# stoneMo/DeepAVFusion

Hardware: AMD Instinct MI355X
Metric: AV-pairs/sec, DeepAVFusion ViT-B pre-training step (224px + 10s audio, image mask 0.75) (higher is better)
Workload: dtype bf16; 1 GPU; AVMAE(DeepAVFusion base) fwd+bwd+allreduce+AdamW, B=64/GPU, 224x224 RGB + (128,640) log-mel, masks 0.75/0.8, fusion attn_ratio 0.25 mlp_ratio 1.0; global_batch=64, parallelism=dp1, graph=True

## Files before the change

deepavfusion_amd/_lib.py:

```python
from __future__ import annotations

import ctypes as C
import os

import torch

_HERE = os.path.dirname(os.path.abspath(__file__))
LIB_PATH = os.path.join(_HERE, 'libdavfusion_hip.so')

_p, _i, _l, _f, _sz = C.c_void_p, C.c_int, C.c_long, C.c_float, C.c_size_t

ABI_VERSION = 9

SIGNATURES = {
    'dav_abi_version': [],
    'dav_build_flags': [],
    'dav_last_error_string': [],
    'dav_tune': [_i, _i],
    'dav_gemm_nt_bf16': [_p, _p, _i, _i, _i, _i, _i, _p, _p, _i, _p, _i, _p, _i, _p, _p, _p, _i, _i, _p, _p, _i, _i, _i, _f, _i, _p],
    'dav_gemm_nt_ln_bf16': [_p, _p, _i, _i, _i, _i, _i, _p, _p, _i, _p, _i, _p, _i, _p, _p, _p, _i, _i, _p, _p, _i, _i, _i, _f, _i, _p, _p],
    'dav_ln_fold_grouped': [_p, _i, _p],
    'dav_rowstats_cast': [_p, _l, _i, _i, _i, _p, _p, _p],
    'dav_layernorm_bwd_twin': [_p, _l, _p, _i, _p, _l, _p, _i, _i, _i, _f, _p, _p, _p, _p,
                               _p, _l, _i, _p, _l, _p, _l,
                               _p, _l, _i, _p, _l, _p, _l,
                               _p, _p, _p, _p, _sz, _p],
    'dav_nt_issue_log': [_i, _p, _i],
    'dav_nt_tune_set': [_p, _i],
    'dav_gemm_tn_bf16': [_p, _p, _i, _i, _i, _i, _i, _p, _p, _p, _i, _i, _p, _i, _p],
    'dav_gemm_tn_grouped_bf16': [_p, _i, _p],
    'dav_gemm_tn_gang_workspace_bytes': [_p, _i],
    'dav_gemm_tn_gang_bf16': [_p, _i, _p, _sz, _p],
    'dav_gemm_tn_grouped_bf16_gated': [_p, _i, _p, _p],
    'dav_gemm_tn_gang_bf16_gated': [_p, _i, _p, _sz, _p, _p],
    'dav_attn_fwd': [_p, _p, _p, _p, _p, _i, _i, _i, _i, _i, _i, _l, _i, _l, _i, _l, _i, _l, _i, _f, _p],
    'dav_attn_bwd': [_p] * 10 + [_i] * 6 + [_l, _i] * 8 + [_f, _p],
    'dav_attn_bwd_part': [_p] * 10 + [_i] * 6 + [_l, _i] * 8 + [_f, _i, _p],
    'dav_add_cast': [_p, _p, _p, _p, _l, _p],
    'dav_attn_bwd_ctx': [_p] * 10 + [_i] * 6 + [_l, _i] * 8 + [_f, _i, _i, _p],
    'dav_attn_bias_fwd': [_p, _p, _p, _p, _p, _i, _i, _i, _i, _i, _i, _l, _i, _l, _i, _l, _i, _l, _i, _f, _p, _i, _i, _p],
    'dav_attn_bias_bwd': [_p] * 10 + [_i] * 6 + [_l, _i] * 8 + [_f, _p, _i, _i, _p, _i, _p],
    'dav_attn_drop_fwd': [_p, _p, _p, _p, _p, _i, _i, _i, _i, _i, _i, _l, _i, _l, _i, _l, _i, _l, _i, _f, _p, _i, _f, _p],
    'dav_attn_drop_bwd': [_p] * 10 + [_i] * 6 + [_l, _i] * 8 + [_f, _p, _i, _f, _i, _i, _p],
    'dav_window_unfold': [_p, _i, _p, _i, _i, _i, _i, _i, _i, _f, _p, _i, _p],
    'dav_window_fold': [_p, _p, _p, _i, _i, _i, _i, _i, _i, _f, _p, _p],
    'dav_relpos_bias_build': [_p, _p, _p, _i, _i, _i, _i, _i, _f, _p, _p],
    'dav_relpos_bias_bwd': [_p, _p, _i, _i, _i, _i, _i, _i, _p, _p],
    'dav_layernorm_fwd': [_p, _l, _i, _p, _l, _i, _i, _i, _p, _p, _f, _p, _p, _p, _p, _p],
    'dav_layernorm_bwd': [_p, _l, _i, _p, _l, _i, _i, _i, _p, _p, _p, _p, _p,
                          _p, _l, _i, _p, _l, _p, _l,
                          _p, _l, _i, _p, _l, _p, _l,
                          _p, _p, _p, _sz, _p],
    'dav_layernorm_bwd_workspace_bytes': [_i, _i],
    'dav_layernorm_bwd_reduce_grouped': [_p, _i, _p],
    'dav_mask_build': [_p, _i, _i, _i, _p, _p, _p, _p, _p, _p],
    'dav_patch_gather': [_p, _i, _i, _i, _i, _p, _i, _p, _p],
    'dav_patch_gather3d': [_p, _i, _i, _i, _i, _i, _i, _p, _i, _p, _p],
    'dav_unshuffle_fwd': [_p, _p, _p, _p, _i, _i, _i, _i, _p, _l, _i, _p],
    'dav_rows_gather_cast': [_p, _l, _i, _p, _i, _i, _i, _p, _p],
    'dav_rows_axpy': [_p, _p, _p, _i, _i, _i, _p, _p],
    'dav_rows_scale_cast': [_p, _p, _i, _i, _i, _p, _p],
    'dav_dropout_rows': [_p, _i, _p, _p, _f, _p, _i, _i, _i, _p, _i, _p],
    'dav_unshuffle_bwd_reduce': [_p, _l, _i, _p, _i, _i, _i, _i, _p, _p, _p],
    'dav_patch_mse_fwd': [_p, _p, _p, _i, _i, _i, _i, _i, _p, _p, _p, _p, _p, _p],
    'dav_patch_mse_bwd': [_p, _p, _p, _p, _p, _p, _p, _i, _i, _i, _i, _p, _p],
    'dav_pair_expand': [_p, _p, _i, _i, _i, _i, _p, _p],
    'dav_pair_reduce': [_p, _i, _i, _i, _i, _p, _p, _p],
    'dav_cast_bf16': [_p, _p, _l, _p],
    'dav_cast_transpose_bf16': [_p, _p, _i, _i, _p],
    'dav_l2norm_workspace_bytes': [_l],
    'dav_l2norm': [_p, _l, _f, _p, _p, _sz, _p],
    'dav_gemm_nt_f32': [_p, _p, _i, _i, _i, _i, _i, _p, _p, _i, _p, _i, _p, _i, _p, _p, _p, _i, _p, _p, _i, _i, _i, _f, _i, _p],
    'dav_gemm_tn_f32': [_p, _p, _i, _i, _i, _i, _i, _p, _p, _p, _i, _i, _p, _p],
    'dav_attn_fwd_f32': [_p, _p, _p, _p, _p, _i, _i, _i, _i, _i, _i, _l, _i, _l, _i, _l, _i, _l, _i, _f, _p],
    'dav_attn_bwd_f32': [_p] * 10 + [_i] * 6 + [_l, _i] * 8 + [_f, _i, _p],
    'dav_attn_bias_fwd_f32': [_p, _p, _p, _p, _p, _i, _i, _i, _i, _i, _i, _l, _i, _l, _i, _l, _i, _l, _i, _f, _p, _i, _i, _p],
    'dav_attn_bias_bwd_f32': [_p] * 10 + [_i] * 6 + [_l, _i] * 8 + [_f, _p, _i, _i, _p, _i, _p],
    'dav_attn_drop_fwd_f32': [_p, _p, _p, _p, _p, _i, _i, _i, _i, _i, _i, _l, _i, _l, _i, _l, _i, _l, _i, _f, _p, _i, _f, _p],
    'dav_attn_drop_bwd_f32': [_p] * 10 + [_i] * 6 + [_l, _i] * 8 + [_f, _p, _i, _f, _i, _p],
    'dav_patch_gather_f32': [_p, _i, _i, _i, _i, _i, _i, _p, _i, _p, _p],
    'dav_rows_gather_f32': [_p, _l, _i, _p, _i, _i, _i, _p, _l, _p],
    'dav_pair_expand_f32': [_p, _p, _i, _i, _i, _i, _p, _p],
    'dav_pair_reduce_f32': [_p, _i, _i, _i, _i, _p, _p, _p],
    'dav_patch_mse_bwd_f32': [_p, _p, _p, _p, _p, _p, _p, _i, _i, _i, _i, _p, _p],
    'dav_add_f32': [_p, _p, _p, _l, _p],
    'dav_logmel': [_p, _i, _i, _i, _i, _i, _p, _p, _p, _p, _p, _p, _f, _i, _i, _p, _p],
    'dav_log10_eps': [_p, _f, _l, _p, _p],
    'dav_mean_l2n_f32': [_p, _i, _i, _i, _l, _l, _p, _p],
    'dav_knn_topk_f32': [_p] * 6 + [_i, _i, _i, _i, _l, _l, _i, _i, _i, _p, _p, _p, _sz, _p],
    'dav_knn_topk_wide_f32': [_p] * 6 + [_i, _i, _i, _i, _l, _l, _i, _i, _i, _p, _p, _p, _sz, _p],
    'dav_knn_vote_f32': [_p, _p, _i, _i, _i, _i, _p, _p, _i, _i, _p, _i, _p, _p, _p],
    'dav_frame_transform_u8': [_p, _i, _i, _i, _p, _i, _f, _f, _f, _f, _f, _f, _p, _p],
    'dav_wave_resample_tile': [_i, _i, _i],
    'dav_wave_resample': [_p, _i, _i, _i, _l, _p, _i, _i, _i, _p, _i, _p, _i, _l, _p],
    'dav_batch_begin': [_i],
    'dav_batch_lane': [],
    'dav_batch_region': [_i],
    'dav_batch_skip': [_i],
    'dav_batch_suspend': [_i],
    'dav_batch_end': [],
    'dav_batch_abort': [],
    'dav_batch_stats': [_p, _p],
    'dav_adamw_flat': [_p, _p, _p, _p, _p, _l, _p, _p, _i, _f, _f, _f, _p, _f, _p, _i, _p, _p, _p],
    'dav_step_guard': [_p, _p, _p, _f, _f, _p, _p, _p],
    'dav_cast_transpose_grouped': [_p, _i, _p],
}

class DavLnReduce(C.Structure):
    _fields_ = [('workspace', C.c_void_p), ('dgamma', C.c_void_p), ('dbeta', C.c_void_p), ('rows', C.c_int), ('D', C.c_int)]


class DavNtLn(C.Structure):
    _fields_ = [('stats', C.c_void_p), ('stats2', C.c_void_p), ('A2', C.c_void_p), ('ln_c', C.c_void_p), ('eps', C.c_float),
                ('a_r0', C.c_int), ('a_r1', C.c_int), ('stats_out', C.c_void_p), ('twin_out', C.c_void_p), ('ld_twin', C.c_int)]


class DavLnFold(C.Structure):
    _fields_ = [('w', C.c_void_p), ('gamma', C.c_void_p), ('beta', C.c_void_p), ('bias', C.c_void_p),
                ('w_ln_bf16', C.c_void_p), ('ln_c', C.c_void_p), ('ln_d', C.c_void_p), ('N', C.c_int), ('K', C.c_int)]


class DavTranspose(C.Structure):
    _fields_ = [('x', C.c_void_p), ('y_bf16', C.c_void_p), ('R', C.c_int), ('C', C.c_int)]


class DavTnProblem(C.Structure):
    _fields_ = [('A', C.c_void_p), ('B', C.c_void_p), ('C', C.c_void_p), ('bias_grad', C.c_void_p),
                ('Mc', C.c_int), ('N', C.c_int), ('K', C.c_int), ('lda', C.c_int), ('ldb', C.c_int), ('ldc', C.c_int),
                ('a_rowmap', C.c_int * 3), ('b_rowmap', C.c_int * 3), ('flags', C.c_int)]


ERRORS = {-1: 'bad shape', -2: 'unsupported dtype', -3: 'insufficient workspace', -4: 'HIP error', -5: 'misaligned pointer/stride'}

_lib = None


def load():
    global _lib
    if _lib is not None:
        return _lib
    if not os.path.exists(LIB_PATH):
        raise RuntimeError(f'{LIB_PATH} is missing: the DeepAVFusion HIP kernels are not built '
                           '(run __graft_entry__.build() or make -C deepavfusion_amd/csrc). There is no CPU fallback.')
    lib = C.CDLL(LIB_PATH)
    for name, argtypes in SIGNATURES.items():
        fn = getattr(lib, name)
        fn.argtypes = argtypes
        fn.restype = _sz if name.endswith('workspace_bytes') else (C.c_char_p if name == 'dav_last_error_string' else _i)
    if lib.dav_abi_version() != ABI_VERSION:
        raise RuntimeError('libdavfusion_hip.so ABI version mismatch')
    _lib = lib
    load_nt_tuning(NT_TUNING_PATH)
    return lib


def kernel_source_hash():
    import glob
    import hashlib
    here = os.path.dirname(os.path.abspath(__file__))
    h = hashlib.sha1()
    for f in sorted(glob.glob(os.path.join(here, 'csrc', '*.hip')) + glob.glob(os.path.join(here, 'csrc', '*.h'))) + [os.path.join(here, 'tuning', 'nt_gfx950.json')]:
        h.update(os.path.basename(f).encode())
        h.update(open(f, 'rb').read())
    return h.hexdigest()[:16]


NT_TUNING_PATH = os.environ.get('DAV_NT_TUNE_FILE') or os.path.join(os.path.dirname(os.path.abspath(__file__)), 'tuning', 'nt_gfx950.json')


def load_nt_tuning(path):
    if os.environ.get('DAV_NT_TUNE', '1') == '0' or not path or not os.path.exists(path):
        _lib.dav_nt_tune_set(None, 0)
        return 0
    import json
    blob = []
    for e in json.load(open(path))['entries']:
        blob += [int(e['cfg']), int(e['b_kn']), len(e['problems'])]
        for q in e['problems']:
            blob += [int(x) for x in q]
    arr = (C.c_int * len(blob))(*blob)
    n = _lib.dav_nt_tune_set(arr, len(blob))
    if n < 0:
        raise RuntimeError(f'{path}: malformed tuning table ({ERRORS.get(n, n)})')
    return n


def check(code: int, what: str):
    if code != 0:
        detail = ''
        if code == -4 and _lib is not None:
            detail = f" ({_lib.dav_last_error_string().decode()})"
        raise RuntimeError(f'{what} failed: {ERRORS.get(code, code)}{detail}')
```

deepavfusion_amd/autograd_bridge.py:

```python
from __future__ import annotations

import os

import torch

from . import engine as E
from . import ops
from .ops import F32


_SIDE_STREAMS = {}


def _streams(dev):
    main = torch.cuda.current_stream(dev)
    if os.environ.get('DAV_STREAMS', '1') == '0':
        return main, main, main
    key = dev.index if dev.index is not None else torch.cuda.current_device()
    if key not in _SIDE_STREAMS:
        _SIDE_STREAMS[key] = (torch.cuda.Stream(dev), torch.cuda.Stream(dev))
    sa, sf = _SIDE_STREAMS[key]
    return main, sa, sf


# ... 270 lines not shown
            E.flush_wgrads()
        if layer_cb is not None and l > 0:
            layer_cb(l)
    E.patch_embed_bwd(vis, t['t_pi'], g_i, g_ib)
    E.patch_embed_bwd(enc.audio, t['t_pa'], g_a, g_ab)
    E.gbuf(enc.fusion_tokens).add_(g_f.sum(dim=0, keepdim=True))
    E._ready(enc.fusion_tokens)


class _EncoderFn(torch.autograd.Function):
    @staticmethod
    def forward(ctx, enc, image, audio, ik32, ak32, return_embs, need_tape, *params):
        ctx.set_materialize_grads(False)
        with E.ln_fuse_for(need_tape):
            _, f32s, embs, tape = encoder_fwd(enc, image, audio, ik32, ak32, want_f32=True, collect_embs=return_embs)
        ctx.enc, ctx.tape = enc, (tape if need_tape else None)
        B = image.shape[0]
        outs = [x.view(B, -1, x.shape[-1]) for x in f32s]
        flat_embs = [e for tri in embs for e in tri]
        ctx.mark_non_differentiable(*flat_embs)
        return (*outs, *flat_embs)

    @staticmethod
    def backward(ctx, gi, ga, gf, *_):
        if ctx.tape is None:
            raise RuntimeError('backward through DeepAVFusion.forward called without a saved tape')
        c = lambda g: None if g is None else g.contiguous().view(-1, g.shape[-1])
        encoder_bwd(ctx.enc, ctx.tape, dxi32=c(gi), dxa32=c(ga), dxf32=c(gf))
        ctx.tape = None
        return (None,) * (7 + len(ctx.enc._param_list))


def encoder_apply(enc, image, audio, image_ids_keep, audio_ids_keep, return_embs):
    enc._param_list = [p for p in enc.parameters()]
    need_tape = torch.is_grad_enabled() and any(p.requires_grad for p in enc._param_list)
    out = _EncoderFn.apply(enc, _f32c(image), _f32c(audio), _ids32(image_ids_keep), _ids32(audio_ids_keep),
                           bool(return_embs), need_tape, *enc._param_list)
    if not return_embs:
        return out[0], out[1], out[2]
    rest = out[3:]
    embs = [tuple(rest[3 * i:3 * i + 3]) for i in range(len(rest) // 3)]
    return out[0], out[1], out[2], embs


class _PatchTokensFn(torch.autograd.Function):
    @staticmethod
    def forward(ctx, vit, x, ids32, *params):
        ctx.set_materialize_grads(False)
        tok, tape = E.patch_embed_fwd(vit, x, ids32)
        ctx.vit, ctx.tape = vit, tape
        return tok

    @staticmethod
    def backward(ctx, g):
        E.patch_embed_bwd(ctx.vit, ctx.tape, g.contiguous(), None)
        return (None,) * (3 + 2)


def patch_tokens(vit, x, ids_keep):
    return _PatchTokensFn.apply(vit, _f32c(x), _ids32(ids_keep), vit.patch_embed.proj.weight, vit.patch_embed.proj.bias)


class _CrossAttentionFn(torch.autograd.Function):

    @staticmethod
    def forward(ctx, ca, x1, x2, *params):
        ctx.set_materialize_grads(False)
        B, N1, D = x1.shape
        N2 = x2.shape[1]
        x1b, x2b = E.to_bf16(x1.reshape(B * N1, D)), E.to_bf16(x2.reshape(B * N2, D))
        H, hd = ca.num_heads, D // ca.num_heads
        S = _sampler(ca, 'cross')
        pa, pp = (ca.attn_drop_prob, ca.proj_drop_prob) if ca.training else (0.0, 0.0)
        keep = E.draw_attn_keep(pa, B, H, N1, N2, x1.device, S('attn', (B, H, N1, N2))) if pa > 0.0 else None
        ctx.pm = E.draw_keep(pp, B * N1, D, x1.device, S('proj', (B, N1, D), lambda m: m.reshape(B * N1, D))) if pp > 0.0 else None
        c = E._cross_fwd_seq(ca, x1b, None, N1, x2b, N2, B, D, ca.num_heads, x1.device, keep=keep)
        out = E.lin_fwd(ca.proj, c['o'], B * N1)
        if ctx.pm is not None:
            E._drop(out, ctx.pm, B, N1, D)
        ctx.ca, ctx.c, ctx.x1b, ctx.x2b, ctx.dims, ctx.np = ca, c, x1b, x2b, (B, N1, N2, D), len(params)
        q = c['q'].view(B, N1, H, hd).permute(0, 2, 1, 3).float()
        k = c['kv'].view(B, N2, 2, H, hd)[:, :, 0].permute(0, 2, 1, 3).float()
        attn = torch.exp((q @ k.transpose(-2, -1)) * ca.scale - c['lse'].unsqueeze(-1))
        if keep is not None:
            attn = attn * keep[0][..., :N2].float() * keep[2]
        ctx.mark_non_differentiable(attn)
        return out.view(B, N1, D), attn

    @staticmethod
    def backward(ctx, g, _g_attn):
        B, N1, N2, D = ctx.dims
        ca = ctx.ca
        with E.deferred_wgrads():
            gb = E.to_bf16(g.contiguous().view(B * N1, D))
            if ctx.pm is not None:
                gb = gb.clone() if gb.data_ptr() == g.data_ptr() else gb
                E._drop(gb, ctx.pm, B, N1, D)
            do = E.lin_bwd(ca.proj, gb, ctx.c['o'], B * N1)
            dx1 = torch.empty(B * N1, D, dtype=E.BF16, device=g.device)
            dx2 = E._cross_bwd_seq(ca, ctx.c, do, ctx.x1b, None, N1, ctx.x2b, N2, B, D, ca.num_heads, dx1, None)
        return (None, dx1.float().view(B, N1, D), dx2.float().view(B, N2, D)) + (None,) * ctx.np


def cross_attention(ca, x1, x2):
    params = [p for p in ca.parameters()]
    c = lambda x: x.to(dtype=F32).contiguous()
    return _CrossAttentionFn.apply(ca, c(x1), c(x2), *params)


class _SwinBlockFn(torch.autograd.Function):
    @staticmethod
    def forward(ctx, blk, xcat, nF, *params):
        ctx.set_materialize_grads(False)
        out, tape = E.swin_block_fwd(blk, xcat, nF)
        ctx.blk, ctx.tape, ctx.np = blk, tape, len(params)
        return out

    @staticmethod
    def backward(ctx, g):
        with E.deferred_wgrads():
            dx, _ = E.swin_block_bwd(ctx.blk, ctx.tape, g.contiguous(), None)
        return (None, dx, None) + (None,) * ctx.np


def swin_block_apply(blk, x, x_fusion):
    nF = x_fusion.shape[1]
    xcat = torch.cat([x_fusion.to(dtype=F32), x.to(dtype=F32)], dim=1).contiguous()
    out = _SwinBlockFn.apply(blk, xcat, nF, *list(blk.parameters()))
    return out[:, nF:], out[:, :nF]


class _FusionBlockFn(torch.autograd.Function):
    @staticmethod
    def forward(ctx, fb, xmm, xv, xa, *params):
        ctx.set_materialize_grads(False)
        out, tape = E.fusion_block_fwd(fb, xmm, xv, xa, fb.num_heads, getattr(fb, 'fusion_tkns', None),
                                       drop_path_scales(fb, fb, xmm.shape[0], xmm.device, 'fusion'),
                                       fusion_drops(fb, fb, xmm.shape[0], xmm.shape[1], xv.shape[1], xa.shape[1], xmm.device, 'fusion'))
        ctx.fb, ctx.tape, ctx.np = fb, tape, len(params)
        return out

    @staticmethod
    def backward(ctx, g):
        with E.deferred_wgrads():
            dx_f, dx_i, dx_a = E.fusion_block_bwd(ctx.fb, ctx.tape, g.contiguous(), None)
        return (None, dx_f, dx_i, dx_a) + (None,) * ctx.np


def fusion_block(fb, xmm, xv, xa):
    c = lambda x: x.to(dtype=F32).contiguous()
    return _FusionBlockFn.apply(fb, c(xmm), c(xv), c(xa), *list(fb.parameters()))


def avmae_fwd(model, image, audio, noise_i, noise_a):
    with E.fold_scope(model):
        return _avmae_fwd(model, image, audio, noise_i, noise_a)


def _avmae_fwd(model, image, audio, noise_i, noise_a):
    enc = model.encoder
    B = image.shape[0]
    Li, La = model.image_gs[0] * model.image_gs[1], model.audio_gs[0] * model.audio_gs[1]
    nki, nka = int(Li * (1 - model.image_mask_ratio)), int(La * (1 - model.audio_mask_ratio))
    ik, im, ir, ik32, ir32 = ops.mask_build(noise_i, nki)
    ak, am, ar, ak32, ar32 = ops.mask_build(noise_a, nka)
    (xi_b, xa_b, xf_b), _, _, t_enc = encoder_fwd(enc, image, audio, ik32, ak32)
    nF = enc.fusion_tokens.shape[1]
    dec_i, dec_a = model.decoder('image'), model.decoder('audio')
    main, sa, _ = _streams(image.device)
    lanes = t_enc['lanes']
    if lanes:
        with E.batch() as bt:
            bt.lane()
            pred_i, t_di = E.decoder_fwd(dec_i, xi_b, xf_b, ir32, B, nki, nF)
            loss_i, t_li = E.loss_fwd(image, pred_i, im, model.image_norm_loss)
            bt.lane()
            pred_a, t_da = E.decoder_fwd(dec_a, xa_b, xf_b, ar32, B, nka, nF)
            loss_a, t_la = E.loss_fwd(audio, pred_a, am, model.audio_norm_loss)
    else:
        si = main
        sa.wait_stream(main)
        if si is not main:
            si.wait_stream(main)

        def chain(dec, x_b, r32, nk, target, mask, norm_loss):
            pred, t_d = yield from E.decoder_fwd_steps(dec, x_b, xf_b, r32, B, nk, nF)
            loss, t_l = E.loss_fwd(target, pred, mask, norm_loss)
            return pred, t_d, loss, t_l
        (pred_a, t_da, loss_a, t_la), (pred_i, t_di, loss_i, t_li) = paired_steps(
            chain(dec_a, xa_b, ar32, nka, audio, am, model.audio_norm_loss), sa,
            chain(dec_i, xi_b, ir32, nki, image, im, model.image_norm_loss), si, DEC_JOIN)
        main.wait_stream(sa)
        if si is not main:
            main.wait_stream(si)
    tape = dict(image=image, audio=audio, im=im, am=am, ik32=ik32, ak32=ak32, dec_lanes=lanes, t_enc=t_enc, t_di=t_di, t_da=t_da, t_li=t_li,
                t_la=t_la, pred_i=pred_i, pred_a=pred_a, B=B)
    aux = dict(image_ids_keep=ik, image_mask=im, image_ids_restore=ir, audio_ids_keep=ak, audio_mask=am, audio_ids_restore=ar)
    return (loss_i, loss_a, pred_i, pred_a), tape, aux


_DEC_WGRAD_JOINT = True
_ADD_CAST = True


def avmae_bwd(model, t, g_li, g_la, g_pi=None, g_pa=None, layer_cb=None):
    B = t['B']
    dec_i, dec_a = model.decoder('image'), model.decoder('audio')
    main, sa, _ = _streams(t['image'].device)
    if t['dec_lanes']:
        dpi = E.loss_bwd(t['image'], t['pred_i'], t['im'], t['t_li'], g_li)
        dpa = E.loss_bwd(t['audio'], t['pred_a'], t['am'], t['t_la'], g_la)
        if g_pi is not None:
            dpi = (dpi.float() + g_pi.reshape(dpi.shape)).to(E.BF16)
        if g_pa is not None:
            dpa = (dpa.float() + g_pa.reshape(dpa.shape)).to(E.BF16)
        with E.deferred_wgrads():
            with E.batch() as bt:
                bt.lane()
                dxi_b, dxf_i = E.decoder_bwd(dec_i, t['t_di'], dpi, t['ik32'], B)
                bt.lane()
                dxa_b, dxf_a = E.decoder_bwd(dec_a, t['t_da'], dpa, t['ak32'], B)
    elif _DEC_WGRAD_JOINT and sa is not main:
        with E.deferred_wgrads():
            si = main
            sa.wait_stream(main)
            if si is not main:
                si.wait_stream(main)

            def chain(dec, target, pred, mask, t_l, g_l, g_p, t_d, k32):
                dp = E.loss_bwd(target, pred, mask, t_l, g_l)
                if g_p is not None:
                    dp = (dp.float() + g_p.reshape(dp.shape)).to(E.BF16)
                return (yield from E.decoder_bwd_steps(dec, t_d, dp, k32, B))
            (dxa_b, dxf_a), (dxi_b, dxf_i) = paired_steps(
                chain(dec_a, t['audio'], t['pred_a'], t['am'], t['t_la'], g_la, g_pa, t['t_da'], t['ak32']), sa,
                chain(dec_i, t['image'], t['pred_i'], t['im'], t['t_li'], g_li, g_pi, t['t_di'], t['ik32']), si, DEC_JOIN)
            main.wait_stream(sa)
            if si is not main:
                main.wait_stream(si)
            E.deferred_operands_to(main)
    else:
        sa.wait_stream(main)
        with torch.cuda.stream(sa), E.deferred_wgrads():
            dpa = E.loss_bwd(t['audio'], t['pred_a'], t['am'], t['t_la'], g_la)
            if g_pa is not None:
                dpa = (dpa.float() + g_pa.reshape(dpa.shape)).to(E.BF16)
            dxa_b, dxf_a = E.decoder_bwd(dec_a, t['t_da'], dpa, t['ak32'], B)
        with E.deferred_wgrads():
            dpi = E.loss_bwd(t['image'], t['pred_i'], t['im'], t['t_li'], g_li)
            if g_pi is not None:
                dpi = (dpi.float() + g_pi.reshape(dpi.shape)).to(E.BF16)
            dxi_b, dxf_i = E.decoder_bwd(dec_i, t['t_di'], dpi, t['ik32'], B)
        main.wait_stream(sa)
    dxf32 = dxf_i.float() + dxf_a.float()
    if layer_cb is not None:
        layer_cb(len(model.encoder.fusion_blocks))
    encoder_bwd(model.encoder, t['t_enc'], dxi_b=dxi_b, dxa_b=dxa_b, dxf32=dxf32, layer_cb=layer_cb)


class _AVMAEFn(torch.autograd.Function):
    @staticmethod
    def forward(ctx, model, image, audio, noise_i, noise_a, need_tape, *params):
        ctx.set_materialize_grads(False)
        with E.ln_fuse_for(need_tape):
            outs, tape, aux = avmae_fwd(model, image, audio, noise_i, noise_a)
        ctx.model, ctx.tape, ctx.np = model, (tape if need_tape else None), len(params)
        model._last_masks = aux
        return outs

    @staticmethod
    def backward(ctx, g_li, g_la, g_pi, g_pa):
        z = lambda g: g.contiguous() if g is not None else torch.zeros((), dtype=F32, device=ctx.tape['image'].device)
        avmae_bwd(ctx.model, ctx.tape, z(g_li), z(g_la), g_pi, g_pa)
        ctx.tape = None
        return (None,) * (6 + ctx.np)


def avmae_apply(model, image, audio, noise_image=None, noise_audio=None):
    B, dev = image.shape[0], image.device
    Li, La = model.image_gs[0] * model.image_gs[1], model.audio_gs[0] * model.audio_gs[1]
    if noise_image is None:
        noise_image = torch.rand(B, Li, device=dev)
    if noise_audio is None:
        noise_audio = torch.rand(B, La, device=dev)
    params = getattr(model, '_param_list', None)
    if params is None:
        params = model._param_list = [p for p in model.parameters()]
    need_tape = torch.is_grad_enabled() and any(p.requires_grad for p in params)
    return _AVMAEFn.apply(model, _f32c(image), _f32c(audio), _f32c(noise_image), _f32c(noise_audio), need_tape, *params)
```

deepavfusion_amd/engine.py:

```python
from __future__ import annotations

import os
from typing import Callable, Dict, List, NamedTuple, Optional

import torch

from . import ops
from .ops import F32

BF16 = torch.bfloat16
PRECISION = 'bf16'


def set_precision(p: str):
    global BF16, PRECISION
    if p not in ('bf16', 'fp32'):
        raise ValueError(p)
    PRECISION = p
    BF16 = torch.float32 if p == 'fp32' else torch.bfloat16

_GRAD_READY: Optional[Callable[[torch.nn.Parameter], None]] = None


def set_grad_ready_hook(fn: Optional[Callable[[torch.nn.Parameter], None]]):
# ... 343 lines not shown
            return self.own.__exit__(et, ev, tb)
        if _BATCH is not None and et is None:
            ops.batch_region(False)
        return False


WGRAD_GANG = os.environ.get('DAV_WGRAD_GANG', '1') != '0'
WGRAD_GANG_MIN_TILES = 512
WGRAD_MERGE = int(os.environ.get('DAV_WGRAD_MERGE', '0'))
WGRAD_FLUSH_LAYERS = None


WGRAD_EAGER_DP_MERGE = 3


def wgrad_flush_due(layer: int, depth: int) -> bool:
    if not WGRAD_GANG or layer == 0 or layer in (WGRAD_FLUSH_LAYERS or ()):
        return True
    if WGRAD_MERGE > 0:
        return (depth - layer) % WGRAD_MERGE == 0
    return _GRAD_READY is not None and WGRAD_FLUSH_LAYERS is None and (depth - layer) % WGRAD_EAGER_DP_MERGE == 0


_DEFERRED = None
_DEFERRED_LN = None
_DEFERRED_LN_READY = []


class deferred_wgrads:
    def __enter__(self):
        global _DEFERRED, _DEFERRED_LN
        self.prev = (_DEFERRED, _DEFERRED_LN)
        _DEFERRED, _DEFERRED_LN = [], []
        return self

    def __exit__(self, *exc):
        global _DEFERRED, _DEFERRED_LN
        if exc[0] is None:
            flush_wgrads()
        _DEFERRED, _DEFERRED_LN = self.prev


_OVERWRITE = None


def wgrad_overwrite_begin(gate=None):
    global _OVERWRITE
    _OVERWRITE = dict(written=set(), touched=set(), params={}, gate=gate)


def wgrad_overwrite_end():
    global _OVERWRITE
    st, _OVERWRITE = _OVERWRITE, None
    return list(st['params'].values()) if st else []


def deferred_operands_to(stream):
    for pr in (_DEFERRED or []):
        for k in ('A', 'B'):
            t = pr.get(k)
            if torch.is_tensor(t) and t.is_cuda:
                t.record_stream(stream)
    for item in (_DEFERRED_LN or []):
        if torch.is_tensor(item[0]) and item[0].is_cuda:
            item[0].record_stream(stream)


def flush_wgrads():
    if _DEFERRED_LN:
        items = list(_DEFERRED_LN)
        del _DEFERRED_LN[:]
        ops.layernorm_bwd_reduce_grouped(items)
        for pair in _DEFERRED_LN_READY:
            _ready(*pair)
        del _DEFERRED_LN_READY[:]
    if not _DEFERRED:
        return
    probs = list(_DEFERRED)
    del _DEFERRED[:]
    while probs:
        seen, now, later = set(), [], []
        for pr in probs:
            key = pr['C'].data_ptr()
            (later if key in seen else now).append(pr)
            seen.add(key)
        now.sort(key=lambda pr: -pr['Mc'])
        gate = _OVERWRITE['gate'] if _OVERWRITE is not None else None
        gated = {} if gate is None else {'gate': gate}
        gang = WGRAD_GANG and PRECISION == 'bf16' and (sum(-(-pr['N'] // 256) * -(-pr['K'] // 256) for pr in now) >= WGRAD_GANG_MIN_TILES
                                                       or any(pr['Mc'] % 64 for pr in now))
        if _OVERWRITE is not None:
            for pr in now:
                key = pr['C'].data_ptr()
                pr['overwrite'] = bool(pr.get('weight') is not None and key not in _OVERWRITE['written'] and key not in _OVERWRITE['touched'])
                if gate is not None and (pr['A'].dtype == F32 or (not gang and pr['Mc'] % 64)):
                    pr['overwrite'] = False
                _OVERWRITE['written'].add(key)
                if pr.get('weight') is None:
                    _OVERWRITE['touched'].add(pr.get('gbase', key))
                if pr['overwrite']:
                    _OVERWRITE['params'][id(pr['weight'])] = pr['weight']
        if gang:
            ops.gemm_tn_gang(now, **gated)
        else:
            grouped = [pr for pr in now if pr['Mc'] % 64 == 0 or pr['A'].dtype == F32]
            if grouped:
                ops.gemm_tn_grouped(grouped, **gated)
            for pr in now:
                if pr['Mc'] % 64 and pr['A'].dtype != F32:
                    ops.gemm_tn(pr['A'], pr['B'], pr['Mc'], pr['N'], pr['K'], pr['C'], lda=pr['lda'], ldb=pr['ldb'], ldc=pr['ldc'],
                                a_rowmap=pr.get('a_rowmap'), b_rowmap=pr.get('b_rowmap'), beta=0 if pr.get('overwrite') else 1,
                                bias_grad=pr.get('bias_grad'))
        for pr in now:
            _ready(*pr['ready'])
        probs = later


def ln_fwd(norm, x0, x1, B, eps=None, want_f32=False, want_bf16=True):
    D = norm.weight.shape[0]
    r0 = x0.shape[1] if x0 is not None else 0
    r1 = x1.shape[1] if x1 is not None else 0
    if x0 is None:
        x0, r0, x1, r1 = x1, r1, None, 0
    dev = x0.device
    M = B * (r0 + r1)
    y = _e((M, D), BF16, dev) if want_bf16 else None
    y32 = _e((M, D), F32, dev) if want_f32 else None
    if PRECISION == 'fp32' and y is not None and y32 is not None:
        y32 = y
    mean, rstd = _e((M,), F32, dev), _e((M,), F32, dev)
    ops.layernorm_fwd(x0, r0 * D, r0, x1, r1 * D, r1, B, D, norm.weight, norm.bias, norm.eps if eps is None else eps,
                      y, y32, mean, rstd)
    return y, y32, (mean, rstd)


def ln_bwd(norm, x0, x1, B, stats, dy_bf16=None, dy_f32=None, *, dx0=None, acc0=0, res0=None, dx0_bf16=None,
           dx1=None, acc1=0, res1=None, dx1_bf16=None):
    D = norm.weight.shape[0]
    r0 = x0.shape[1] if x0 is not None else 0
    r1 = x1.shape[1] if x1 is not None else 0
    if x0 is None:
        x0, r0, x1, r1 = x1, r1, None, 0
        dx0, acc0, res0, dx0_bf16, dx1, acc1, res1, dx1_bf16 = dx1, acc1, res1, dx1_bf16, None, 0, None, None
    ops.layernorm_bwd(x0, r0 * D, r0, x1, r1 * D, r1, B, D, dy_bf16, dy_f32, norm.weight, stats[0], stats[1],
                      dx0, r0 * D, acc0, res0, r0 * D, dx0_bf16, r0 * D,
                      dx1, r1 * D, acc1, res1, r1 * D, dx1_bf16, r1 * D,
                      gbuf(norm.weight), gbuf(norm.bias), defer=_DEFERRED_LN)
    if _DEFERRED_LN is None:
        _ready(norm.weight, norm.bias)
    else:
        _DEFERRED_LN_READY.append((norm.weight, norm.bias))


def lin_fwd(lin, a, M, *, a_rowmap=None, lda=None, act=0, res=None, res_rowmap=None, out=None, out_bf16=False,
            c_rowmap=None, ldc=None, C2=None, c2_mode=0, w_col_off=0, k=None, use_bias=True):
    W = wcache(lin.weight)
    N, Kfull = W.shape
    K = Kfull if k is None else k
    dev = a.device
    if out is None:
        out = _e((M, N), BF16 if out_bf16 else F32, dev)
    Bw = W if w_col_off == 0 else W.view(-1)[w_col_off:]
    ops.gemm_nt(a, Bw, M, N, K, lda=lda if lda is not None else K, ldb=Kfull, a_rowmap=a_rowmap,
                bias=lin.bias if use_bias else None, act=act, res=res, ldres=N, res_rowmap=res_rowmap,
                C_out=out, ldc=ldc if ldc is not None else N, c_bf16=out.dtype == BF16, c_rowmap=c_rowmap,
                C2=C2, ldc2=N, c2_mode=c2_mode)
    return out


def lin_bwd(lin, dy, a, M, *, dy_rowmap=None, a_rowmap=None, lda=None, need_dx=True, gelu_aux=None, dx=None, dx_bf16=True,
            dx_rowmap=None, dx_beta=0, dx_C2=None, dx_c2_mode=0, w_col_off=0, k=None, use_bias=True, final=True,
            dx_res=None, dx_res_rowmap=None, wgrad=True):
    W = wcache(lin.weight)
    N, Kfull = W.shape
    K = Kfull if k is None else k
    dev = dy.device
    if need_dx:
        if dx is None:
            dx = _e((M, K), BF16 if dx_bf16 else F32, dev)
        if N % 64 == 0 or PRECISION == 'fp32':
            Bt, ldb, variant = (W if w_col_off == 0 else W.view(-1)[w_col_off:]), Kfull, 1 << 12
        else:
            WT = wcache_t(lin.weight)
            Bt, ldb, variant = (WT if w_col_off == 0 else WT[w_col_off:]), N, 0
        ops.gemm_nt(dy, Bt, M, K, N, lda=N, ldb=ldb, a_rowmap=dy_rowmap, act=3 if gelu_aux is not None else 0,
                    aux=gelu_aux, ldaux=K, res=dx_res, ldres=K, res_rowmap=dx_res_rowmap,
                    C_out=dx, ldc=K, c_bf16=dx.dtype == BF16, c_rowmap=dx_rowmap, beta=dx_beta,
                    C2=dx_C2, ldc2=K, c2_mode=dx_c2_mode, variant=variant)
    if wgrad:
        lin_wgrad(lin, dy, a, M, dy_rowmap=dy_rowmap, a_rowmap=a_rowmap, lda=lda, w_col_off=w_col_off, k=k, use_bias=use_bias, final=final)
    return dx


def lin_wgrad(lin, dy, a, M, *, dy_rowmap=None, a_rowmap=None, lda=None, w_col_off=0, k=None, use_bias=True, final=True):
    N, Kfull = lin.weight.shape[0], lin.weight.numel() // lin.weight.shape[0]
    K = Kfull if k is None else k
    gw = gbuf(lin.weight)
    gwv = gw.view(N, -1)
    Cw = gwv if w_col_off == 0 else gwv.view(-1)[w_col_off:]
    gb = gbuf(lin.bias) if (use_bias and lin.bias is not None) else None
    if _DEFERRED is not None and N % 8 == 0 and K % 8 == 0 and (M % 64 == 0 or (WGRAD_GANG and PRECISION == 'bf16')):
        _DEFERRED.append(dict(A=dy, B=a, Mc=M, N=N, K=K, C=Cw, lda=N, ldb=lda if lda is not None else K, ldc=Kfull,
                              a_rowmap=dy_rowmap, b_rowmap=a_rowmap, bias_grad=gb,
                              ready=(lin.weight, lin.bias) if final else (),
                              gbase=gwv.data_ptr(),
                              weight=lin.weight if (w_col_off == 0 and K == Kfull) else None))
        return
    if _OVERWRITE is not None:
        _OVERWRITE['touched'].add(gwv.data_ptr())
    ops.gemm_tn(dy, a, M, N, K, Cw, lda=N, ldb=lda if lda is not None else K, ldc=Kfull, a_rowmap=dy_rowmap,
                b_rowmap=a_rowmap, beta=1, bias_grad=gb)
    if final:
        _ready(lin.weight, lin.bias)


def lin_fwd_ln(lin, norm, eps, t0, M, *, t1=None, r0=0, r1=0, a_rowmap=None, act=0, out_bf16=True, out=None, C2=None, c2_mode=0):
    f = ln_fold(lin, norm)
    N, K = f.wl.shape
    if out is None:
        out = _e((M, N), BF16 if out_bf16 else F32, f.wl.device)
    ln = dict(stats=t0[1], ln_c=f.c, eps=eps)
    if t1 is not None:
        ln.update(A2=t1[0], stats2=t1[1], a_r0=r0, a_r1=r1)
    ops.gemm_nt_ln(t0[0], f.wl, M, N, K, ln=ln, a_rowmap=a_rowmap, bias=f.d, act=act, C_out=out, c_bf16=out.dtype == BF16,
                   C2=C2, ldc2=N, c2_mode=c2_mode)
    return out


def lin_fwd_tw(lin, a, M, res, *, res_rowmap=None, res_rows=None, out=None, tw=None, c_rowmap=None, C2=None, c2_mode=0, rows_out=None):
    W = wcache(lin.weight)
    N, K = W.shape
    dev = a.device
    R = M if rows_out is None else rows_out
    if out is None:
        out = _e((R, N), F32, dev)
    if tw is None:
        tw = (_e((R, N), BF16, dev), _e((R, N // 64, 2), F32, dev))
    ops.gemm_nt_ln(a, W, M, N, K, prod=dict(stats_out=tw[1], twin_out=tw[0], ld_twin=N), bias=lin.bias, res=res, ldres=N,
                   res_rowmap=res_rowmap, res_rows=res_rows, C_out=out, c_rowmap=c_rowmap, C2=C2, ldc2=N, c2_mode=c2_mode)
    return out, tw


def ln_bwd_tw(norm, eps, t0, r0, t1, r1, B, dy_bf16=None, dy_f32=None, *, h_out=None, dx0=None, acc0=0, res0=None, dx0_bf16=None,
              dx1=None, acc1=0, res1=None, dx1_bf16=None):
    D = norm.weight.shape[0]
    if t0 is None:
        t0, r0, t1, r1 = t1, r1, None, 0
        dx0, acc0, res0, dx0_bf16, dx1, acc1, res1, dx1_bf16 = dx1, acc1, res1, dx1_bf16, None, 0, None, None
    ops.layernorm_bwd_twin(t0[0], r0 * D, t0[1], r0, t1[0] if t1 is not None else None, r1 * D, t1[1] if t1 is not None else None, r1,
                           B, D, eps, dy_bf16, dy_f32, norm.weight, norm.bias,
                           dx0, r0 * D, acc0, res0, r0 * D, dx0_bf16, r0 * D,
                           dx1, r1 * D, acc1, res1, r1 * D, dx1_bf16, r1 * D,
                           h_out=h_out, dgamma=gbuf(norm.weight), dbeta=gbuf(norm.bias), defer=_DEFERRED_LN)
    if _DEFERRED_LN is None:
        _ready(norm.weight, norm.bias)
    else:
        _DEFERRED_LN_READY.append((norm.weight, norm.bias))


class AttnView(NamedTuple):
    t: torch.Tensor
    off: int
    bs: int
    rs: int


def cols(buf, rows, c0=0, r0=0):
    ld = buf.shape[1]
    return AttnView(buf, r0 * ld + c0, rows * ld, ld)


def qkv_cols(qkv, rows, D, r0=0):
    return cols(qkv, rows, 0, r0), cols(qkv, rows, D), cols(qkv, rows, 2 * D)


def _attn_ptr(name, v, B, N, width, r0_is=0):
    t, off, bs, rs = v
    ok = t.dim() == 2 and t.is_contiguous() and off >= 0 and rs == t.shape[1] and rs > 0 and bs % rs == 0 and t.shape[0] == B * (bs // rs)
    if ok:
        r0, c0 = divmod(off, rs)
        ok = c0 + width <= rs and r0 + N <= bs // rs and (not r0_is or r0 == r0_is)
    if not ok:
        raise ValueError(f'attention operand {name}: (off, bs, rs) = {tuple(v[1:])} into {tuple(t.shape)} (contiguous: {t.is_contiguous()}) '
                         f'does not hold {B} x {N} rows of {width} columns' + (f' from row {r0_is}' if r0_is else ''))
    return t.data_ptr() + t.element_size() * off


def attention_fwd(q, k, v, B, H, Nq, Nk, dqk, dv, scale, keep=None, bias=None):
    ptrs = (_attn_ptr('q', q, B, Nq, H * dqk), _attn_ptr('k', k, B, Nk, H * dqk), _attn_ptr('v', v, B, Nk, H * dv))
    dev = q.t.device
    O = _e((B * Nq, H * dv), BF16, dev)
    LSE = _e((B, H, Nq), F32, dev)
    ops.hold(q.t, k.t, v.t)
    args = (*ptrs, O, LSE, B, H, Nq, Nk, dqk, dv, q.bs, q.rs, k.bs, k.rs, v.bs, v.rs, Nq * H * dv, H * dv, scale)
    if keep is not None:
        ops.attn_drop_fwd(*args, *keep)
    elif bias is not None:
        ops.attn_bias_fwd(*args, *bias)
    else:
        ops.attn_fwd(*args)
    return O, LSE


_ATTN_CTX = True


def attention_bwd(q, k, v, O, dO, LSE, dq, dk, dv_, B, H, Nq, Nk, dqk, dv, scale, part=3, Delta=None, dq_ctx_rows=0, keep=None,
                  bias=None, dS=None):
    ptrs = (_attn_ptr('q', q, B, Nq, H * dqk), _attn_ptr('k', k, B, Nk, H * dqk), _attn_ptr('v', v, B, Nk, H * dv),
            _attn_ptr('dq', dq, B, Nq, H * dqk, dq_ctx_rows), _attn_ptr('dk', dk, B, Nk, H * dqk), _attn_ptr('dv', dv_, B, Nk, H * dv))
    if Delta is None:
        Delta = torch.empty_like(LSE)
    ops.hold(q.t, k.t, v.t, dq.t, dk.t, dv_.t)
    args = (*ptrs[:3], O, dO, LSE, Delta, *ptrs[3:], B, H, Nq, Nk, dqk, dv, q.bs, q.rs, k.bs, k.rs, v.bs, v.rs,
            Nq * H * dv, H * dv, Nq * H * dv, H * dv, dq.bs, dq.rs, dk.bs, dk.rs, dv_.bs, dv_.rs, scale)
    if keep is not None:
        ops.attn_drop_bwd(*args, *keep, part=part, dq_ctx_rows=dq_ctx_rows)
    elif bias is not None:
        ops.attn_bias_bwd(*args, *bias, dS, part=part)
    else:
        ops.attn_bwd(*args, part=part, dq_ctx_rows=dq_ctx_rows)


def to_bf16(x):
    if PRECISION == 'fp32':
        return x.contiguous()
    y = torch.empty(x.shape, dtype=BF16, device=x.device)
    ops.cast_bf16(x.contiguous(), y)
    return y


def draw_attn_keep(p, B, H, Nq, Nk, dev, sample=None):
    ld = (Nk + 31) // 32 * 32
    if sample is None:
        m = (torch.rand((B, H, Nq, ld), device=dev) >= p).to(torch.uint8)
    else:
        m = torch.zeros((B, H, Nq, ld), device=dev, dtype=torch.uint8)
# ... 535 lines not shown
    B, nF, D = x_f.shape
    n2, n3 = x_2.shape[1], x_3.shape[1]
    nS = n3 + n2
    dev, at = x_f.device, fb.attn
    Da = at.q.weight.shape[0]
    hd = Da // heads
    g1, g1b = _mlp_tail_bwd(fb, t, g, gb, B, nF, D, dev)
    dp, dr = t.get('dp'), t.get('dr') or {}
    if dp is not None or 'proj' in dr:
        g1b = _branch_grad(g1, None if dp is None else dp[0], dr.get('proj'), B, nF, D)
    do = lin_bwd(at.proj, g1b, t['o'], B * nF)
    dq, dkv = _e((B * nF, Da), BF16, dev), _e((B * nS, 2 * Da), BF16, dev)
    attention_bwd(cols(t['q'], nF), cols(t['kv'], nS), cols(t['kv'], nS, Da), t['o'], do, t['lse'],
                  cols(dq, nF), cols(dkv, nS), cols(dkv, nS, Da), B, heads, nF, nS, hd, hd, hd ** -0.5, keep=dr.get('attn'))
    dxmm_b = lin_bwd(at.q, dq, t['xmm_b'], B * nF)
    dx3_b = lin_bwd(at.kv, dkv, t['x3_b'], B * n3, dy_rowmap=(n3, nS, 0), final=False)
    dx2_b = lin_bwd(at.kv, dkv, t['x2_b'], B * n2, dy_rowmap=(n2, nS, n3))
    return _input_norms_bwd(fb, t, (fb.norm1_aud, x_2, t['st_2'], dx2_b), (fb.norm1_img, x_3, t['st_3'], dx3_b), dxmm_b, g1, dx_i, dx_a)


def _dense_fwd(fb, x_f, x_i, x_a, heads, dp=None, dr=None):
    dr = dr or {}
    B, nF, D = x_f.shape
    nI, nA = x_i.shape[1], x_a.shape[1]
    dev, at = x_f.device, fb.attn
    Da = at.q.weight.shape[0]
    hd = Da // heads
    xmm_b, xmm32, st_mm = ln_fwd(fb.norm1_mm, None, x_f, B, want_f32=True)
    xi_b, _, st_i = ln_fwd(fb.norm1_img, None, x_i, B)
    xa_b, _, st_a = ln_fwd(fb.norm1_aud, None, x_a, B)
    pa = lin_fwd(at.kv, xa_b, B * nA, k=D)
    pi = lin_fwd(at.kv, xi_b, B * nI, k=D, w_col_off=D, use_bias=False)
    P = nA * nI
    KV = _e((B * P, 2 * Da), BF16, dev)
    ops.pair_expand(pa, pi, B, nA, nI, 2 * Da, KV)
    q = lin_fwd(at.q, xmm_b, B * nF, out_bf16=True)
    scale = (D // heads) ** -0.5
    o, lse = attention_fwd(cols(q, nF), cols(KV, P), cols(KV, P, Da), B, heads, nF, P, hd, hd, scale, keep=dr.get('attn'))
    xmm1 = _res_add(at.proj, o, B * nF, xmm32, B, nF, D, None if dp is None else dp[0], drop=dr.get('proj')).view(B, nF, D)
    out, tt = _mlp_tail_fwd(fb, xmm1, B, nF, D, dev, dp, dr)
    tt.update(arch='dense_mmi', x_f=x_f, x_i=x_i, x_a=x_a, xmm_b=xmm_b, st_mm=st_mm, xi_b=xi_b, st_i=st_i, xa_b=xa_b, st_a=st_a,
              KV=KV, q=q, o=o, lse=lse, heads=heads)
    return out, tt


def _dense_bwd(fb, t, g, gb, *, dx_i=None, dx_a=None):
    x_f, x_i, x_a, heads = t['x_f'], t['x_i'], t['x_a'], t['heads']
    B, nF, D = x_f.shape
    nI, nA = x_i.shape[1], x_a.shape[1]
    P = nA * nI
    dev, at = x_f.device, fb.attn
    Da = at.q.weight.shape[0]
    hd = Da // heads
    g1, g1b = _mlp_tail_bwd(fb, t, g, gb, B, nF, D, dev)
    dp, dr = t.get('dp'), t.get('dr') or {}
    if dp is not None or 'proj' in dr:
        g1b = _branch_grad(g1, None if dp is None else dp[0], dr.get('proj'), B, nF, D)
    do = lin_bwd(at.proj, g1b, t['o'], B * nF)
    dq, dKV = _e((B * nF, Da), BF16, dev), _e((B * P, 2 * Da), BF16, dev)
    scale = (D // heads) ** -0.5
    attention_bwd(cols(t['q'], nF), cols(t['KV'], P), cols(t['KV'], P, Da), t['o'], do, t['lse'],
                  cols(dq, nF), cols(dKV, P), cols(dKV, P, Da), B, heads, nF, P, hd, hd, scale, keep=dr.get('attn'))
    dxmm_b = lin_bwd(at.q, dq, t['xmm_b'], B * nF)
    dpa, dpi = _e((B * nA, 2 * Da), BF16, dev), _e((B * nI, 2 * Da), BF16, dev)
    ops.pair_reduce(dKV, B, nA, nI, 2 * Da, dpa, dpi)
    dxa_b = lin_bwd(at.kv, dpa, t['xa_b'], B * nA, k=D, final=False)
    dxi_b = lin_bwd(at.kv, dpi, t['xi_b'], B * nI, k=D, w_col_off=D, use_bias=False)
    return _input_norms_bwd(fb, t, (fb.norm1_img, x_i, t['st_i'], dxi_b), (fb.norm1_aud, x_a, t['st_a'], dxa_b), dxmm_b, g1, dx_i, dx_a)


FUSION_IDLE_FWD, FUSION_IDLE_BWD = 4, 6



def fusion_block_batchable(fb, dp=None, dr=None):
    return dp is None and not dr and getattr(fb, 'arch', 'factorized_mmi') == 'factorized_mmi'


def fusion_block_fwd(fb, x_f, x_i, x_a, heads, tkns, dp=None, dr=None):
    arch = getattr(fb, 'arch', 'factorized_mmi')
    if arch == 'token':
        return _token_fwd(fb, x_f, x_i, x_a, heads, dp, dr)
    if arch == 'dense_mmi':
        return _dense_fwd(fb, x_f, x_i, x_a, heads, dp, dr)
    return _factorized_fwd(fb, x_f, x_i, x_a, heads, tkns, dp, dr)


def fusion_block_bwd(fb, t, g, gb, *, dx_i=None, dx_a=None):
    arch = t.get('arch', 'factorized_mmi')
    if arch == 'token':
        return _token_bwd(fb, t, g, gb, dx_i=dx_i, dx_a=dx_a)
    if arch == 'dense_mmi':
        return _dense_bwd(fb, t, g, gb, dx_i=dx_i, dx_a=dx_a)
    return _factorized_bwd(fb, t, g, gb, dx_i=dx_i, dx_a=dx_a)


def patch_embed_fwd(vit, img, ids_keep32):
    B, C = img.shape[:2]
    pe = vit.patch_embed
    L = pe.num_patches
    nk = ids_keep32.shape[1] if ids_keep32 is not None else L
    D = vit.embed_dim
    clip = img.dim() == 5
    pt = pe.patch_size[0] if clip else 1
    if not clip:
        H, W = img.shape[2], img.shape[3]
        assert H == pe.img_size[0], f"Input image height ({H}) doesn't match model ({pe.img_size[0]})."
        assert W == pe.img_size[1], f"Input image width ({W}) doesn't match model ({pe.img_size[1]})."
    else:
        got = (img.shape[2] // pt) * (img.shape[3] // 16) * (img.shape[4] // 16)
        if tuple(img.shape[2:]) != tuple(pe.input_size):
            raise RuntimeError(f'The size of tensor a ({got}) must match the size of tensor b ({L}) at non-singleton dimension 1')
    if C != pe.proj.weight.shape[1]:
        raise RuntimeError(f'Given groups=1, weight of size {list(pe.proj.weight.shape)}, expected input{list(img.shape)} to have '
                           f'{pe.proj.weight.shape[1]} channels, but got {C} channels instead')
    if clip and nk != L:
        raise RuntimeError(f'The size of tensor a ({nk}) must match the size of tensor b ({L}) at non-singleton dimension 1')
    K = C * pt * 256
    A = _e((B * nk, K), BF16, img.device)
    ops.patch_gather(img, ids_keep32, nk, A, pt)
    Wb = wcache(pe.proj.weight)
    tok = _e((B, nk, D), F32, img.device)
    pos_by_id = ids_keep32 is not None and not clip
    if ln_fuse_ok(D) and K % 64 == 0:
        tw = (_e((B * nk, D), BF16, img.device), _e((B * nk, D // 64, 2), F32, img.device))
        ops.gemm_nt_ln(A, Wb, B * nk, D, K, prod=dict(stats_out=tw[1], twin_out=tw[0], ld_twin=D), bias=pe.proj.bias, res=vit.pos_embed,
                       ldres=D, res_rows=ids_keep32 if pos_by_id else None, res_rowmap=None if pos_by_id else (L, 0, 0), C_out=tok)
        tw_set(tok, *tw)
    else:
        ops.gemm_nt(A, Wb, B * nk, D, K, bias=pe.proj.bias, res=vit.pos_embed, ldres=D,
                    res_rows=ids_keep32 if pos_by_id else None, res_rowmap=None if pos_by_id else (L, 0, 0), C_out=tok)
    return tok, dict(A=A, nk=nk)


def patch_embed_bwd(vit, t, g, gb):
    pe = vit.patch_embed
    D = vit.embed_dim
    A = t['A']
    M, K = A.shape
    if gb is None:
        gb = to_bf16(g)
    ops.gemm_tn(gb, A, M, D, K, gbuf(pe.proj.weight).view(D, K), beta=1, bias_grad=gbuf(pe.proj.bias))
    _ready(pe.proj.weight, pe.proj.bias)


def drain(steps):
    try:
        while True:
            next(steps)
    except StopIteration as e:
        return e.value


def decoder_fwd(dec, x_b, xf_b, ids_restore32, B, nk, nF):
    return drain(decoder_fwd_steps(dec, x_b, xf_b, ids_restore32, B, nk, nF))


def decoder_fwd_steps(dec, x_b, xf_b, ids_restore32, B, nk, nF):
    L = ids_restore32.shape[1]
    Dd = dec.embed.weight.shape[0]
    dev = x_b.device
    emb = lin_fwd(dec.embed, x_b, B * nk)
    x = _e((B, nF + L, Dd), F32, dev)
    lin_fwd(dec.embed, xf_b, B * nF, out=x, c_rowmap=(nF, nF + L, 0))
    ops.unshuffle_fwd(emb, dec.mask_token, dec.pos_embed, ids_restore32, B, L, nk, Dd, x, (nF + L) * Dd, nF)
    tapes = []
    swin = getattr(dec, 'arch', 'plain') == 'swin'
    for blk in dec.blocks:
        if swin:
            x, bt = swin_block_fwd(blk, x, nF)
        else:
            x, bt = block_fwd(blk, x, None, dec.heads, blk.norm1.eps)
        tapes.append(bt)
        yield
    D_ = Dd
    if not swin and ln_fuse_ok(Dd):
        tw_last = ensure_tw(x)
        pred = lin_fwd_ln(dec.pred, dec.norm, dec.norm.eps, tw_last, B * L, a_rowmap=(L, nF + L, nF), out_bf16=False)
        P = pred.shape[1]
        tape = dict(x_b=x_b, xf_b=xf_b, tapes=tapes, tw_last=tw_last, ln_fused=True, ids_restore32=ids_restore32, nk=nk, nF=nF, L=L)
        return pred.view(B, L, P), tape
    hN = _e((B * L, D_), BF16, dev)
    mean, rstd = _e((B * L,), F32, dev), _e((B * L,), F32, dev)
    xs = x.view(-1)[nF * Dd:]
    ops.layernorm_fwd(xs, (nF + L) * Dd, L, None, 0, 0, B, Dd, dec.norm.weight, dec.norm.bias, dec.norm.eps, hN, None, mean, rstd)
    pred = lin_fwd(dec.pred, hN, B * L)
    P = pred.shape[1]
    tape = dict(x_b=x_b, xf_b=xf_b, x_last=x, tapes=tapes, hN=hN, stN=(mean, rstd), ids_restore32=ids_restore32, nk=nk, nF=nF, L=L)
    return pred.view(B, L, P), tape


def decoder_bwd(dec, t, dpred_b, ids_keep32, B):
    return drain(decoder_bwd_steps(dec, t, dpred_b, ids_keep32, B))


def decoder_bwd_steps(dec, t, dpred_b, ids_keep32, B):
    nk, nF, L = t['nk'], t['nF'], t['L']
    Dd = dec.embed.weight.shape[0]
    dev = dpred_b.device
    fused = t.get('ln_fused', False)
    dhN = lin_bwd(dec.pred, dpred_b, None if fused else t['hN'], B * L, wgrad=not fused)
    g = _e((B, nF + L, Dd), F32, dev)
    gb = _e((B * (nF + L), Dd), BF16, dev)
    g[:, :nF].zero_()
    gb.view(B, nF + L, Dd)[:, :nF].zero_()
    if fused:
        xb, st = t['tw_last']
        hN = _e((B * L, Dd), BF16, dev)
        ops.layernorm_bwd_twin((xb, nF * Dd), (nF + L) * Dd, (st, nF * (Dd // 64) * 2), L, None, 0, None, 0, B, Dd, dec.norm.eps,
                               dhN, None, dec.norm.weight, dec.norm.bias,
                               (g, nF * Dd), (nF + L) * Dd, 0, None, 0, (gb, nF * Dd), (nF + L) * Dd,
                               h_out=hN, dgamma=gbuf(dec.norm.weight), dbeta=gbuf(dec.norm.bias))
        lin_wgrad(dec.pred, dpred_b, hN, B * L)
    else:
        xs = t['x_last'].view(-1)[nF * Dd:]
        ops.layernorm_bwd(xs, (nF + L) * Dd, L, None, 0, 0, B, Dd, dhN, None, dec.norm.weight, t['stN'][0], t['stN'][1],
                          g.view(-1)[nF * Dd:], (nF + L) * Dd, 0, None, 0, gb.view(-1)[nF * Dd:], (nF + L) * Dd,
                          None, 0, 0, None, 0, None, 0, gbuf(dec.norm.weight), gbuf(dec.norm.bias))
    _ready(dec.norm.weight, dec.norm.bias)
    swin = getattr(dec, 'arch', 'plain') == 'swin'
    yield
    for blk, bt in zip(reversed(list(dec.blocks)), reversed(t['tapes'])):
        if swin:
            g, gb = swin_block_bwd(blk, bt, g, gb)
        else:
            g, gb, _ = block_bwd(blk, bt, g, gb)
        yield
    d_emb = _e((B * nk, Dd), BF16, dev)
    d_embf = _e((B * nF, Dd), BF16, dev)
    ops.rows_gather_cast(g, (nF + L) * Dd, nF, ids_keep32, B, nk, Dd, d_emb)
    ops.rows_gather_cast(g, (nF + L) * Dd, 0, None, B, nF, Dd, d_embf)
    ops.unshuffle_bwd_reduce(g, (nF + L) * Dd, nF, t['ids_restore32'], B, L, nk, Dd, gbuf(dec.pos_embed), gbuf(dec.mask_token))
    _ready(dec.pos_embed, dec.mask_token)
    dx_b = lin_bwd(dec.embed, d_emb, t['x_b'], B * nk, final=False)
    dxf_b = lin_bwd(dec.embed, d_embf, t['xf_b'], B * nF)
    return dx_b, dxf_b


LOG2E = 1.4426950408889634


def swin_block_fwd(blk, x, nF):
    B, R, D = x.shape
    L, dev = R - nF, x.device
    heads, nW = blk.num_heads, blk.num_windows
    A = blk.attn.window_area
    N, hd, M, Mw = A + nF, D // heads, B * R, B * nW * (A + nF)
    h1, _, st1 = ln_fwd(blk.norm1, None, x, B)
    seq = _e((Mw, D), BF16, dev)
    ops.window_unfold(h1, blk.rows32, B, nW, A, nF, L, D, 1.0, seq)
    qkv = lin_fwd(blk.attn.qkv, seq, Mw, out_bf16=True)
    nb = nW if blk.attn_mask is not None else 1
    ld = (N + 31) // 32 * 32
    bias = _e((nb, heads, N, ld), F32, dev)
    ops.relpos_bias_build(blk.attn.relative_position_bias_table, blk.index32, blk.attn_mask, nb, heads, A, N, ld,
                          1.0 if PRECISION == 'fp32' else LOG2E, bias)
    o, lse = attention_fwd(*qkv_cols(qkv, N, D), B * nW, heads, N, N, hd, hd, blk.attn.scale, bias=(bias, nb, ld))
    t = lin_fwd(blk.attn.proj, o, Mw)
    x1 = _e((B, R, D), F32, dev)
    ops.window_fold(t, blk.inv32, x, B, nW, A, nF, L, D, 1.0 / nW, x1)
    h2, _, st2 = ln_fwd(blk.norm2, None, x1, B)
    Hd = blk.mlp.fc1.weight.shape[0]
    z = _e((M, Hd), BF16, dev)
    u = lin_fwd(blk.mlp.fc1, h2, M, act=1, out_bf16=True, C2=z, c2_mode=4)
    x2 = _res_add(blk.mlp.fc2, u, M, x1, B, R, D, None).view(B, R, D)
    tape = dict(x=x, nF=nF, h1=h1, st1=st1, seq=seq, qkv=qkv, bias=bias, nb=nb, ld=ld, o=o, lse=lse, x1=x1, h2=h2, st2=st2, z=z, u=u)
    return x2, tape


def swin_block_bwd(blk, t, g2, g2b=None):
    x, nF = t['x'], t['nF']
    B, R, D = x.shape
    L, dev = R - nF, x.device
    heads, nW = blk.num_heads, blk.num_windows
    A = blk.attn.window_area
    N, hd, M, Mw = A + nF, D // heads, B * R, B * nW * (A + nF)
    if g2b is None:
        g2b = to_bf16(g2.view(M, D))
    dz = lin_bwd(blk.mlp.fc2, g2b, t['u'], M, gelu_aux=t['z'])
    dh2 = lin_bwd(blk.mlp.fc1, dz, t['h2'], M)
    g1 = _e((B, R, D), F32, dev)
    ln_bwd(blk.norm2, None, t['x1'], B, t['st2'], dy_bf16=dh2, dx1=g1, res1=g2)
    dt = _e((Mw, D), BF16, dev)
    ops.window_unfold(g1, blk.rows32, B, nW, A, nF, L, D, 1.0 / nW, dt)
    do = lin_bwd(blk.attn.proj, dt, t['o'], Mw)
    dqkv = _e((Mw, 3 * D), BF16, dev)
    dS = _e((B * nW, heads, N, t['ld']), F32, dev)
    attention_bwd(*qkv_cols(t['qkv'], N, D), t['o'], do, t['lse'], *qkv_cols(dqkv, N, D), B * nW, heads, N, N, hd, hd, blk.attn.scale,
                  bias=(t['bias'], t['nb'], t['ld']), dS=dS)
    table = blk.attn.relative_position_bias_table
    ops.relpos_bias_bwd(dS, blk.index32, B * nW, heads, A, N, t['ld'], table.shape[0], gbuf(table))
    _ready(table)
    dseq = lin_bwd(blk.attn.qkv, dqkv, t['seq'], Mw, dx_bf16=False)
    dh1 = _e((M, D), F32, dev)
    ops.window_fold(dseq, blk.inv32, None, B, nW, A, nF, L, D, 1.0, dh1)
    dx = _e((B, R, D), F32, dev)
    dxb = _e((M, D), BF16, dev)
    ln_bwd(blk.norm1, None, x, B, t['st1'], dy_f32=dh1, dx1=dx, res1=g1, dx1_bf16=dxb)
    return dx, dxb


def loss_fwd(img, pred, mask, norm_pix):
    B, L = mask.shape
    dev = img.device
    lp, tm, tr = _e((B * L,), F32, dev), _e((B * L,), F32, dev), _e((B * L,), F32, dev)
    loss, msum = _e((1,), F32, dev), _e((1,), F32, dev)
    ops.patch_mse_fwd(img, pred, mask, norm_pix, lp, tm, tr, loss, msum)
    return loss.view(()), dict(tm=tm, tr=tr, msum=msum)


def loss_bwd(img, pred, mask, t, gout):
    B, L, P = pred.shape
    dpred = _e((B * L, P), BF16, img.device)
    ops.patch_mse_bwd(img, pred, mask, t['tm'], t['tr'], t['msum'], gout, dpred)
    return dpred
```

deepavfusion_amd/ops.py:

```python
from __future__ import annotations

import ctypes as C
from typing import Optional, Sequence

import torch

from . import _lib

BF16 = torch.bfloat16
F32 = torch.float32


def _stream():
    return torch.cuda.current_stream().cuda_stream


import threading

_TLS = threading.local()


def hold(*tensors):
    h = getattr(_TLS, 'hold', None)
    if h is not None:
# ... 4 lines not shown
    if t is None:
        return None
    if not t.is_cuda:
        raise RuntimeError('deepavfusion_amd kernels need tensors on an MI355X (cuda) device; there is no CPU fallback')
    h = getattr(_TLS, 'hold', None)
    if h is not None:
        h.append(t)
    return t.data_ptr()


def batch_begin(auto_lanes=False):
    _lib.check(_lib.load().dav_batch_begin(int(auto_lanes)), 'dav_batch_begin')
    _TLS.hold = []


def batch_lane():
    _lib.check(_lib.load().dav_batch_lane(), 'dav_batch_lane')


def batch_skip(steps):
    _lib.check(_lib.load().dav_batch_skip(int(steps)), 'dav_batch_skip')


def batch_region(begin):
    _lib.check(_lib.load().dav_batch_region(int(begin)), 'dav_batch_region')


class unbatched:

    def __enter__(self):
        self.on = getattr(_TLS, 'hold', None) is not None
        if self.on:
            _lib.load().dav_batch_suspend(1)

    def __exit__(self, *exc):
        if self.on:
            _lib.load().dav_batch_suspend(0)
        return False


def batch_end(abort=False):
    lib = _lib.load()
    try:
        if abort:
            lib.dav_batch_abort()
            return 0, 0
        _lib.check(lib.dav_batch_end(), 'dav_batch_end')
        a, b = C.c_int(0), C.c_int(0)
        lib.dav_batch_stats(C.byref(a), C.byref(b))
        return a.value, b.value
    finally:
        _TLS.hold = None


def _rm(m: Optional[Sequence[int]]):
    return (C.c_int * 3)(*m) if m is not None else None


def gemm_nt(A, B, M, N, K, *, lda=None, ldb=None, a_rowmap=None, bias=None, act=0, aux=None, ldaux=0, res=None, ldres=0,
            res_rowmap=None, res_rows=None, C_out=None, ldc=None, c_bf16=False, c_rowmap=None, C2=None, ldc2=0, c2_mode=0,
            beta=0, alpha=1.0, variant=0):
    lib = _lib.load()
    if A.dtype == F32:
        _lib.check(lib.dav_gemm_nt_f32(_ptr(A), _ptr(B), M, N, K, lda if lda is not None else K, ldb if ldb is not None else K,
                                       _rm(a_rowmap), _ptr(bias), act, _ptr(aux), ldaux, _ptr(res), ldres, _rm(res_rowmap),
                                       _ptr(res_rows), _ptr(C_out), ldc if ldc is not None else N, _rm(c_rowmap), _ptr(C2), ldc2,
                                       c2_mode, beta, float(alpha), (variant >> 12) & 1, _stream()), 'dav_gemm_nt_f32')
        return
    _lib.check(lib.dav_gemm_nt_bf16(_ptr(A), _ptr(B), M, N, K, lda if lda is not None else K, ldb if ldb is not None else K,
                                    _rm(a_rowmap), _ptr(bias), act, _ptr(aux), ldaux, _ptr(res), ldres, _rm(res_rowmap),
                                    _ptr(res_rows), _ptr(C_out), ldc if ldc is not None else N, int(c_bf16), _rm(c_rowmap),
                                    _ptr(C2), ldc2, c2_mode, beta, float(alpha), variant, _stream()), 'dav_gemm_nt_bf16')


def gemm_nt_ln(A, B, M, N, K, *, ln=None, prod=None, lda=None, ldb=None, a_rowmap=None, bias=None, act=0, aux=None, ldaux=0, res=None,
               ldres=0, res_rowmap=None, res_rows=None, C_out=None, ldc=None, c_bf16=False, c_rowmap=None, C2=None, ldc2=0,
               c2_mode=0, beta=0, variant=0):
    lib = _lib.load()
    q = _lib.DavNtLn()
    if ln is not None:
        q.stats, q.ln_c, q.eps = _ptr(ln['stats']), _ptr(ln['ln_c']), float(ln['eps'])
        q.stats2, q.A2 = _ptr(ln.get('stats2')), _ptr(ln.get('A2'))
        q.a_r0, q.a_r1 = int(ln.get('a_r0', 0)), int(ln.get('a_r1', 0))
    if prod is not None:
        q.stats_out, q.twin_out, q.ld_twin = _ptr(prod.get('stats_out')), _ptr(prod.get('twin_out')), int(prod.get('ld_twin', N))
    _lib.check(lib.dav_gemm_nt_ln_bf16(_ptr(A), _ptr(B), M, N, K, lda if lda is not None else K, ldb if ldb is not None else K,
                                       _rm(a_rowmap), _ptr(bias), act, _ptr(aux), ldaux, _ptr(res), ldres, _rm(res_rowmap),
                                       _ptr(res_rows), _ptr(C_out), ldc if ldc is not None else N, int(c_bf16), _rm(c_rowmap),
                                       _ptr(C2), ldc2, c2_mode, beta, 1.0, variant, C.byref(q), _stream()), 'dav_gemm_nt_ln_bf16')


LN_FOLD_MAX = 48


def ln_fold_grouped(items):
    lib = _lib.load()
    for i in range(0, len(items), LN_FOLD_MAX):
        chunk = items[i:i + LN_FOLD_MAX]
        arr = (_lib.DavLnFold * len(chunk))()
        for q, (w, g, b, bias, wl, c, d) in zip(arr, chunk):
            q.w, q.gamma, q.beta, q.bias, q.w_ln_bf16, q.ln_c, q.ln_d = _ptr(w), _ptr(g), _ptr(b), _ptr(bias), _ptr(wl), _ptr(c), _ptr(d)
            q.N, q.K = int(w.shape[0]), int(w.shape[1])
        _lib.check(lib.dav_ln_fold_grouped(arr, len(chunk), _stream()), 'dav_ln_fold_grouped')


def rowstats_cast(x, x_bs, B, rows, D, twin, stats):
    _lib.check(_lib.load().dav_rowstats_cast(_ptr(x), x_bs, B, rows, D, _ptr(twin), _ptr(stats), _stream()), 'dav_rowstats_cast')


def layernorm_bwd_twin(xb0, xb0_bs, st0, r0, xb1, xb1_bs, st1, r1, B, D, eps, dy_bf16, dy_f32, gamma, beta,
                       dx0=None, dx0_bs=0, acc0=0, res0=None, res0_bs=0, dx0_bf16=None, dx0_bf_bs=0,
                       dx1=None, dx1_bs=0, acc1=0, res1=None, res1_bs=0, dx1_bf16=None, dx1_bf_bs=0, h_out=None, dgamma=None, dbeta=None,
                       defer=None):
    lib = _lib.load()

    def po(t):
        if t is None:
            return None
        if isinstance(t, tuple):
            return _ptr(t[0]) + t[0].element_size() * t[1]
        return _ptr(t)
    ws = None
    if dgamma is not None:
        ws = torch.empty(lib.dav_layernorm_bwd_workspace_bytes(B * (r0 + r1), D) // 4, dtype=F32, device=dgamma.device)
        if defer is not None:
            defer.append((ws, dgamma, dbeta, B * (r0 + r1), D))
            dgamma = dbeta = None
    _lib.check(lib.dav_layernorm_bwd_twin(po(xb0), xb0_bs, po(st0), r0, po(xb1), xb1_bs, po(st1), r1, B, D, float(eps),
                                          _ptr(dy_bf16), _ptr(dy_f32), _ptr(gamma), _ptr(beta),
                                          po(dx0), dx0_bs, acc0, po(res0), res0_bs, po(dx0_bf16), dx0_bf_bs,
                                          po(dx1), dx1_bs, acc1, po(res1), res1_bs, po(dx1_bf16), dx1_bf_bs,
                                          _ptr(h_out), _ptr(dgamma), _ptr(dbeta), _ptr(ws), ws.numel() * 4 if ws is not None else 0,
                                          _stream()), 'dav_layernorm_bwd_twin')


def nt_issue_log(enable=None, with_flags=False):
    lib = _lib.load()
    if enable is not None:
        lib.dav_nt_issue_log(int(enable), None, 0)
        return None
    n = -lib.dav_nt_issue_log(0, (C.c_int * 1)(), 0)
    if n <= 0:
        return []
    buf = (C.c_int * n)()
    lib.dav_nt_issue_log(0, buf, n)
    out, i = [], 0
    while i < n:
        cfg, bt, cnt = buf[i], buf[i + 1], buf[i + 2]
        probs = [(buf[i + 3 + 4 * j], buf[i + 4 + 4 * j], buf[i + 5 + 4 * j]) for j in range(cnt)]
        flags = [buf[i + 6 + 4 * j] for j in range(cnt)]
        out.append((cfg, bt, probs, flags) if with_flags else (cfg, bt, probs))
        i += 3 + 4 * cnt
    return out


def gemm_tn(A, B, Mc, N, K, C_out, *, lda=None, ldb=None, ldc=None, a_rowmap=None, b_rowmap=None, beta=1, bias_grad=None,
            variant=0):
    lib = _lib.load()
    if A.dtype == F32:
        _lib.check(lib.dav_gemm_tn_f32(_ptr(A), _ptr(B), Mc, N, K, lda if lda is not None else N, ldb if ldb is not None else K,
                                       _rm(a_rowmap), _rm(b_rowmap), _ptr(C_out), ldc if ldc is not None else K, beta,
                                       _ptr(bias_grad), _stream()), 'dav_gemm_tn_f32')
        return
    _lib.check(lib.dav_gemm_tn_bf16(_ptr(A), _ptr(B), Mc, N, K, lda if lda is not None else N, ldb if ldb is not None else K,
                                    _rm(a_rowmap), _rm(b_rowmap), _ptr(C_out), ldc if ldc is not None else K, beta,
                                    _ptr(bias_grad), variant, _stream()), 'dav_gemm_tn_bf16')


TN_GROUP_MAX = 40


def _gate_ptr(gate):
    if gate.dtype != torch.int32 or gate.numel() != 1 or not gate.is_cuda:
        raise ValueError('write gate: one int32 element in device memory')
    return _ptr(gate)


def gemm_tn_grouped(problems, gate=None):
    lib = _lib.load()
    if problems and problems[0]['A'].dtype == F32:
        if gate is not None and any(d.get('overwrite') for d in problems):
            raise RuntimeError('gemm_tn_grouped: the fp32 path has no gated form; queue its problems without overwrite')
        for d in problems:
            gemm_tn(d['A'], d['B'], d['Mc'], d['N'], d['K'], d['C'], lda=d['lda'], ldb=d['ldb'], ldc=d['ldc'],
                    a_rowmap=d.get('a_rowmap'), b_rowmap=d.get('b_rowmap'), beta=0 if d.get('overwrite') else 1,
                    bias_grad=d.get('bias_grad'))
        return
    n_launch = (len(problems) + TN_GROUP_MAX - 1) // TN_GROUP_MAX
    for i in range(n_launch):
        chunk = problems[i::n_launch]
        if gate is not None:
            _lib.check(lib.dav_gemm_tn_grouped_bf16_gated(_tn_problem_array(chunk), len(chunk), _gate_ptr(gate), _stream()),
                       'dav_gemm_tn_grouped_bf16_gated')
            continue
        _lib.check(lib.dav_gemm_tn_grouped_bf16(_tn_problem_array(chunk), len(chunk), _stream()), 'dav_gemm_tn_grouped_bf16')


def _tn_problem_array(problems):
    arr = (_lib.DavTnProblem * len(problems))()
    for q, d in zip(arr, problems):
        q.A, q.B, q.C, q.bias_grad = _ptr(d['A']), _ptr(d['B']), _ptr(d['C']), _ptr(d.get('bias_grad'))
        q.Mc, q.N, q.K, q.lda, q.ldb, q.ldc = d['Mc'], d['N'], d['K'], d['lda'], d['ldb'], d['ldc']
        q.a_rowmap[:] = d.get('a_rowmap') or (0, 0, 0)
        q.b_rowmap[:] = d.get('b_rowmap') or (0, 0, 0)
        q.flags = 1 if d.get('overwrite') else 0
    return arr


def gemm_tn_gang(problems, workspace_fill=None, gate=None):
    if not problems:
        return
    if problems[0]['A'].dtype == F32:
        return gemm_tn_grouped(problems) if gate is None else gemm_tn_grouped(problems, gate)
    lib = _lib.load()
    arr = _tn_problem_array(problems)
    nbytes = int(lib.dav_gemm_tn_gang_workspace_bytes(arr, len(problems)))
    if nbytes == 0:
        raise RuntimeError('dav_gemm_tn_gang_workspace_bytes: invalid weight-gradient problem (shape / alignment)')
    ws = torch.empty(nbytes, dtype=torch.uint8, device=problems[0]['A'].device)
    if workspace_fill is not None:
        ws.fill_(workspace_fill)
    hold(ws)
    if gate is not None:
        _lib.check(lib.dav_gemm_tn_gang_bf16_gated(arr, len(problems), _ptr(ws), nbytes, _gate_ptr(gate), _stream()), 'dav_gemm_tn_gang_bf16_gated')
        return
    _lib.check(lib.dav_gemm_tn_gang_bf16(arr, len(problems), _ptr(ws), nbytes, _stream()), 'dav_gemm_tn_gang_bf16')


def _attn_fwd_call(variant, q_ptr, k_ptr, v_ptr, O, LSE, dims, scale, tail=()):
    name = 'dav_attn' + variant + '_fwd' + ('_f32' if O.dtype == F32 else '')
    _lib.check(getattr(_lib.load(), name)(q_ptr, k_ptr, v_ptr, _ptr(O), _ptr(LSE), *dims, float(scale), *tail, _stream()), name)


def _attn_bwd_call(variant, q_ptr, k_ptr, v_ptr, O, dO, LSE, Delta, dq_ptr, dk_ptr, dv_ptr, dims, scale, part, tail=(), dq_ctx_rows=0):
    f32 = O.dtype == F32
    if variant == '':
        entry = 'dav_attn_bwd_f32' if f32 else ('dav_attn_bwd_ctx' if dq_ctx_rows else 'dav_attn_bwd_part')
    else:
        entry = 'dav_attn' + variant + '_bwd' + ('_f32' if f32 else '')
    ctx = (int(dq_ctx_rows),) if entry in ('dav_attn_bwd_ctx', 'dav_attn_drop_bwd') else ()
    _lib.check(getattr(_lib.load(), entry)(q_ptr, k_ptr, v_ptr, _ptr(O), _ptr(dO), _ptr(LSE), _ptr(Delta), dq_ptr, dk_ptr, dv_ptr, *dims,
                                           float(scale), *tail, *ctx, part, _stream()),
               'dav_attn_bwd' if entry == 'dav_attn_bwd_part' else entry)


def attn_fwd(q_ptr, k_ptr, v_ptr, O, LSE, B, H, Nq, Nk, dqk, dv, q_bs, q_rs, k_bs, k_rs, v_bs, v_rs, o_bs, o_rs, scale):
    _attn_fwd_call('', q_ptr, k_ptr, v_ptr, O, LSE, (B, H, Nq, Nk, dqk, dv, q_bs, q_rs, k_bs, k_rs, v_bs, v_rs, o_bs, o_rs), scale)


def attn_bias_fwd(q_ptr, k_ptr, v_ptr, O, LSE, B, H, Nq, Nk, dqk, dv, q_bs, q_rs, k_bs, k_rs, v_bs, v_rs, o_bs, o_rs, scale,
                  bias, bias_nb, bias_ld):
    _attn_fwd_call('_bias', q_ptr, k_ptr, v_ptr, O, LSE, (B, H, Nq, Nk, dqk, dv, q_bs, q_rs, k_bs, k_rs, v_bs, v_rs, o_bs, o_rs), scale,
                   (_ptr(bias), bias_nb, bias_ld))


def attn_bias_bwd(q_ptr, k_ptr, v_ptr, O, dO, LSE, Delta, dq_ptr, dk_ptr, dv_ptr, B, H, Nq, Nk, dqk, dv, q_bs, q_rs, k_bs, k_rs,
                  v_bs, v_rs, o_bs, o_rs, do_bs, do_rs, dq_bs, dq_rs, dk_bs, dk_rs, dv_bs, dv_rs, scale, bias, bias_nb, bias_ld,
                  dS, part=3):
    _attn_bwd_call('_bias', q_ptr, k_ptr, v_ptr, O, dO, LSE, Delta, dq_ptr, dk_ptr, dv_ptr,
                   (B, H, Nq, Nk, dqk, dv, q_bs, q_rs, k_bs, k_rs, v_bs, v_rs, o_bs, o_rs, do_bs, do_rs, dq_bs, dq_rs, dk_bs, dk_rs,
                    dv_bs, dv_rs), scale, part, (_ptr(bias), bias_nb, bias_ld, _ptr(dS)))


def window_unfold(src, rows32, B, nW, A, nF, L, Cc, fusion_scale, out):
    _lib.check(_lib.load().dav_window_unfold(_ptr(src), int(src.dtype == BF16), _ptr(rows32), B, nW, A, nF, L, Cc, float(fusion_scale),
                                             _ptr(out), int(out.dtype == BF16), _stream()), 'dav_window_unfold')


def window_fold(t, inv32, res, B, nW, A, nF, L, Cc, fusion_scale, out):
    _lib.check(_lib.load().dav_window_fold(_ptr(t), _ptr(inv32), _ptr(res), B, nW, A, nF, L, Cc, float(fusion_scale), _ptr(out),
                                           _stream()), 'dav_window_fold')


def relpos_bias_build(table, index32, mask, nb, H, A, N, ld, mul, out):
    _lib.check(_lib.load().dav_relpos_bias_build(_ptr(table), _ptr(index32), _ptr(mask), nb, H, A, N, ld, float(mul), _ptr(out),
                                                 _stream()), 'dav_relpos_bias_build')


def relpos_bias_bwd(dS, index32, Bw, H, A, N, ld, T, dtable):
    _lib.check(_lib.load().dav_relpos_bias_bwd(_ptr(dS), _ptr(index32), Bw, H, A, N, ld, T, _ptr(dtable), _stream()),
               'dav_relpos_bias_bwd')


def attn_bwd(q_ptr, k_ptr, v_ptr, O, dO, LSE, Delta, dq_ptr, dk_ptr, dv_ptr, B, H, Nq, Nk, dqk, dv, q_bs, q_rs, k_bs, k_rs,
             v_bs, v_rs, o_bs, o_rs, do_bs, do_rs, dq_bs, dq_rs, dk_bs, dk_rs, dv_bs, dv_rs, scale, part=3, dq_ctx_rows=0):
    if O.dtype == F32 and dq_ctx_rows:
        raise RuntimeError('dq_ctx_rows: bf16 path only')
    _attn_bwd_call('', q_ptr, k_ptr, v_ptr, O, dO, LSE, Delta, dq_ptr, dk_ptr, dv_ptr,
                   (B, H, Nq, Nk, dqk, dv, q_bs, q_rs, k_bs, k_rs, v_bs, v_rs, o_bs, o_rs, do_bs, do_rs, dq_bs, dq_rs, dk_bs, dk_rs,
                    dv_bs, dv_rs), scale, part, dq_ctx_rows=dq_ctx_rows)


ATTN_RESIDENT_MAX = 80 * 1024


def attn_bwd_onepass_lds(Nq, Nk, dqk, dv):
    nqp, nkp = (Nq + 31) & ~31, (Nk + 31) & ~31
    return nqp * (2 * max(dqk, 32) + 2 * max(dv, 32)) + nkp * 2 * max(dqk, 32) + nqp * nkp * 2 + nqp * 8


def attn_bwd_onepass_fits(Nq, Nk, dqk, dv):
    return (dqk, dv) in ((64, 64), (16, 64)) and attn_bwd_onepass_lds(Nq, Nk, dqk, dv) <= ATTN_RESIDENT_MAX


def layernorm_fwd(x0, x0_bs, r0, x1, x1_bs, r1, B, D, gamma, beta, eps, y_bf16, y_f32, mean, rstd):
    lib = _lib.load()
    if y_bf16 is not None and y_bf16.dtype == F32:
        if y_f32 is not None and y_f32.data_ptr() != y_bf16.data_ptr():
            raise RuntimeError('fp32 LayerNorm: pass one output buffer')
        y_bf16, y_f32 = None, y_bf16
    _lib.check(lib.dav_layernorm_fwd(_ptr(x0), x0_bs, r0, _ptr(x1), x1_bs, r1, B, D, _ptr(gamma), _ptr(beta), float(eps),
                                     _ptr(y_bf16), _ptr(y_f32), _ptr(mean), _ptr(rstd), _stream()), 'dav_layernorm_fwd')


def layernorm_bwd(x0, x0_bs, r0, x1, x1_bs, r1, B, D, dy_bf16, dy_f32, gamma, mean, rstd,
                  dx0=None, dx0_bs=0, acc0=0, res0=None, res0_bs=0, dx0_bf16=None, dx0_bf_bs=0,
                  dx1=None, dx1_bs=0, acc1=0, res1=None, res1_bs=0, dx1_bf16=None, dx1_bf_bs=0, dgamma=None, dbeta=None,
                  defer=None):
    lib = _lib.load()
    twins = []
    if dy_bf16 is not None and dy_bf16.dtype == F32:
        if dy_f32 is not None:
            tmp = torch.empty_like(dy_bf16)
            _lib.check(lib.dav_add_f32(_ptr(dy_bf16), _ptr(dy_f32), _ptr(tmp), tmp.numel(), _stream()), 'dav_add_f32')
            dy_f32 = tmp
        else:
            dy_f32 = dy_bf16
        dy_bf16 = None
    if dx0_bf16 is not None and dx0_bf16.dtype == F32:
        twins.append((dx0, dx0_bs, r0, dx0_bf16, dx0_bf_bs))
        dx0_bf16 = None
    if dx1_bf16 is not None and dx1_bf16.dtype == F32:
        twins.append((dx1, dx1_bs, r1, dx1_bf16, dx1_bf_bs))
        dx1_bf16 = None
    ws = None
    if dgamma is not None:
        ws = torch.empty(lib.dav_layernorm_bwd_workspace_bytes(B * (r0 + r1), D) // 4, dtype=F32, device=dgamma.device)
        if defer is not None:
            defer.append((ws, dgamma, dbeta, B * (r0 + r1), D))
            dgamma = dbeta = None
    _lib.check(lib.dav_layernorm_bwd(_ptr(x0), x0_bs, r0, _ptr(x1), x1_bs, r1, B, D, _ptr(dy_bf16), _ptr(dy_f32),
                                     _ptr(gamma), _ptr(mean), _ptr(rstd),
                                     _ptr(dx0), dx0_bs, acc0, _ptr(res0), res0_bs, _ptr(dx0_bf16), dx0_bf_bs,
                                     _ptr(dx1), dx1_bs, acc1, _ptr(res1), res1_bs, _ptr(dx1_bf16), dx1_bf_bs,
                                     _ptr(dgamma), _ptr(dbeta), _ptr(ws), ws.numel() * 4 if ws is not None else 0, _stream()),
               'dav_layernorm_bwd')
    for (dx, bs, rows, twin, twin_bs) in twins:
        _lib.check(lib.dav_rows_gather_f32(_ptr(dx), bs, 0, None, B, rows, D, _ptr(twin), twin_bs, _stream()), 'dav_rows_gather_f32')


def layernorm_bwd_reduce_grouped(items):
    lib = _lib.load()
    for i in range(0, len(items), 64):
        chunk = items[i:i + 64]
        arr = (_lib.DavLnReduce * len(chunk))()
        for q, (ws, dg, db, rows, D) in zip(arr, chunk):
            q.workspace, q.dgamma, q.dbeta, q.rows, q.D = _ptr(ws), _ptr(dg), _ptr(db), rows, D
        _lib.check(lib.dav_layernorm_bwd_reduce_grouped(arr, len(chunk), _stream()), 'dav_layernorm_bwd_reduce_grouped')


def mask_build(noise: torch.Tensor, len_keep: int):
    lib = _lib.load()
    N, L = noise.shape
    dev = noise.device
    ids_keep = torch.empty(N, len_keep, dtype=torch.int64, device=dev)
    ids_restore = torch.empty(N, L, dtype=torch.int64, device=dev)
    mask = torch.empty(N, L, dtype=F32, device=dev)
    ids_keep32 = torch.empty(N, len_keep, dtype=torch.int32, device=dev)
    ids_restore32 = torch.empty(N, L, dtype=torch.int32, device=dev)
    _lib.check(lib.dav_mask_build(_ptr(noise.contiguous()), N, L, len_keep, _ptr(ids_keep), _ptr(ids_restore), _ptr(mask),
                                  _ptr(ids_keep32), _ptr(ids_restore32), _stream()), 'dav_mask_build')
    return ids_keep, mask, ids_restore, ids_keep32, ids_restore32


def patch_gather(img, ids_keep32, nk, out, pt=1):
    lib = _lib.load()
    if out.dtype == F32:
        if img.dim() == 5:
            B, Cc, T, H, W = img.shape
        else:
            (B, Cc, H, W), T = img.shape, 1
        _lib.check(lib.dav_patch_gather_f32(_ptr(img), B, Cc, T, H, W, pt, _ptr(ids_keep32), nk, _ptr(out), _stream()), 'dav_patch_gather_f32')
        return
    if img.dim() == 5:
        B, Cc, T, H, W = img.shape
        _lib.check(lib.dav_patch_gather3d(_ptr(img), B, Cc, T, H, W, pt, _ptr(ids_keep32), nk, _ptr(out), _stream()),
                   'dav_patch_gather3d')
        return
    B, Cc, H, W = img.shape
    _lib.check(lib.dav_patch_gather(_ptr(img), B, Cc, H, W, _ptr(ids_keep32), nk, _ptr(out), _stream()), 'dav_patch_gather')


def unshuffle_fwd(emb, mask_token, pos, ids_restore32, B, L, nk, D, out, out_bs, out_row_off):
    lib = _lib.load()
    _lib.check(lib.dav_unshuffle_fwd(_ptr(emb), _ptr(mask_token), _ptr(pos), _ptr(ids_restore32), B, L, nk, D, _ptr(out),
                                     out_bs, out_row_off, _stream()), 'dav_unshuffle_fwd')


def rows_gather_cast(x, x_bs, row_off, ids32, B, n, D, out):
    lib = _lib.load()
    if out.dtype == F32:
        _lib.check(lib.dav_rows_gather_f32(_ptr(x), x_bs, row_off, _ptr(ids32), B, n, D, _ptr(out), 0, _stream()), 'dav_rows_gather_f32')
        return
    _lib.check(lib.dav_rows_gather_cast(_ptr(x), x_bs, row_off, _ptr(ids32), B, n, D, _ptr(out), _stream()), 'dav_rows_gather_cast')


def unshuffle_bwd_reduce(dx, dx_bs, row_off, ids_restore32, B, L, nk, D, dpos, dmask_token):
    lib = _lib.load()
    _lib.check(lib.dav_unshuffle_bwd_reduce(_ptr(dx), dx_bs, row_off, _ptr(ids_restore32), B, L, nk, D, _ptr(dpos),
                                            _ptr(dmask_token), _stream()), 'dav_unshuffle_bwd_reduce')


def patch_mse_fwd(img, pred, mask, norm_pix, loss_patch, tmean, trstd, loss, mask_sum):
    lib = _lib.load()
    B, Cc, H, W = img.shape
    _lib.check(lib.dav_patch_mse_fwd(_ptr(img), _ptr(pred), _ptr(mask), B, Cc, H, W, int(norm_pix), _ptr(loss_patch),
                                     _ptr(tmean), _ptr(trstd), _ptr(loss), _ptr(mask_sum), _stream()), 'dav_patch_mse_fwd')


def patch_mse_bwd(img, pred, mask, tmean, trstd, mask_sum, gout, dpred_bf16):
    lib = _lib.load()
    B, Cc, H, W = img.shape
    if dpred_bf16.dtype == F32:
        _lib.check(lib.dav_patch_mse_bwd_f32(_ptr(img), _ptr(pred), _ptr(mask), _ptr(tmean), _ptr(trstd), _ptr(mask_sum), _ptr(gout),
                                             B, Cc, H, W, _ptr(dpred_bf16), _stream()), 'dav_patch_mse_bwd_f32')
        return
    _lib.check(lib.dav_patch_mse_bwd(_ptr(img), _ptr(pred), _ptr(mask), _ptr(tmean), _ptr(trstd), _ptr(mask_sum), _ptr(gout),
                                     B, Cc, H, W, _ptr(dpred_bf16), _stream()), 'dav_patch_mse_bwd')


def pair_expand(Pv, Pa, B, nv, na, Wd, out):
    lib = _lib.load()
    if out.dtype == F32:
        _lib.check(lib.dav_pair_expand_f32(_ptr(Pv), _ptr(Pa), B, nv, na, Wd, _ptr(out), _stream()), 'dav_pair_expand_f32')
        return
    _lib.check(lib.dav_pair_expand(_ptr(Pv), _ptr(Pa), B, nv, na, Wd, _ptr(out), _stream()), 'dav_pair_expand')


def pair_reduce(d, B, nv, na, Wd, dPv, dPa):
    lib = _lib.load()
    if d.dtype == F32:
        _lib.check(lib.dav_pair_reduce_f32(_ptr(d), B, nv, na, Wd, _ptr(dPv), _ptr(dPa), _stream()), 'dav_pair_reduce_f32')
        return
    _lib.check(lib.dav_pair_reduce(_ptr(d), B, nv, na, Wd, _ptr(dPv), _ptr(dPa), _stream()), 'dav_pair_reduce')


def cast_bf16(x, y):
    lib = _lib.load()
    _lib.check(lib.dav_cast_bf16(_ptr(x), _ptr(y), x.numel(), _stream()), 'dav_cast_bf16')


def cast_transpose_bf16(x2d, y):
    lib = _lib.load()
    R, Cc = x2d.shape
    _lib.check(lib.dav_cast_transpose_bf16(_ptr(x2d), _ptr(y), R, Cc, _stream()), 'dav_cast_transpose_bf16')


def l2norm(x_flat, out, workspace, scale=1.0):
    lib = _lib.load()
    _lib.check(lib.dav_l2norm(_ptr(x_flat), x_flat.numel(), float(scale), _ptr(out), _ptr(workspace),
                              workspace.numel() * workspace.element_size(), _stream()), 'dav_l2norm')


def adamw_flat(p, g, m, v, p_bf16, seg_end, hyper, nseg, beta1, beta2, eps, bias_corr, grad_scale=1.0, sumsq_out=None,
               zero_grad=False, keep_grad=None, gscale_dev=None):
    lib = _lib.load()
    _lib.check(lib.dav_adamw_flat(_ptr(p), _ptr(g), _ptr(m), _ptr(v), _ptr(p_bf16), p.numel(), _ptr(seg_end), _ptr(hyper), nseg,
                                  float(beta1), float(beta2), float(eps), _ptr(bias_corr), float(grad_scale), _ptr(sumsq_out),
                                  int(zero_grad), _ptr(keep_grad), _ptr(gscale_dev), _stream()), 'dav_adamw_flat')


def add_cast(a, b):
    lib = _lib.load()
    out = torch.empty_like(a)
    out_b = torch.empty(a.shape, dtype=BF16, device=a.device)
    _lib.check(lib.dav_add_cast(_ptr(a), _ptr(b), _ptr(out), _ptr(out_b), a.numel(), _stream()), 'dav_add_cast')
    return out, out_b


def step_guard(loss_a, loss_b, gnorm, clip, grad_scale, out_scale, bad_count):
    lib = _lib.load()
    _lib.check(lib.dav_step_guard(_ptr(loss_a), _ptr(loss_b), _ptr(gnorm), float(clip if clip else 0.0), float(grad_scale),
                                  _ptr(out_scale), _ptr(bad_count), _stream()), 'dav_step_guard')


def rows_axpy(res, y, scale, B, rows, D, out):
    lib = _lib.load()
    _lib.check(lib.dav_rows_axpy(_ptr(res), _ptr(y), _ptr(scale), B, rows, D, _ptr(out), _stream()), 'dav_rows_axpy')


def rows_scale_cast(g, scale, B, rows, D, out_bf16):
    lib = _lib.load()
    _lib.check(lib.dav_rows_scale_cast(_ptr(g), _ptr(scale), B, rows, D, _ptr(out_bf16), _stream()), 'dav_rows_scale_cast')


def attn_drop_fwd(q_ptr, k_ptr, v_ptr, O, LSE, B, H, Nq, Nk, dqk, dv, q_bs, q_rs, k_bs, k_rs, v_bs, v_rs, o_bs, o_rs, scale,
                  keep, keep_ld, keep_scale):
    _attn_fwd_call('_drop', q_ptr, k_ptr, v_ptr, O, LSE, (B, H, Nq, Nk, dqk, dv, q_bs, q_rs, k_bs, k_rs, v_bs, v_rs, o_bs, o_rs), scale,
                   (_ptr(keep), keep_ld, float(keep_scale)))


def attn_drop_bwd(q_ptr, k_ptr, v_ptr, O, dO, LSE, Delta, dq_ptr, dk_ptr, dv_ptr, B, H, Nq, Nk, dqk, dv, q_bs, q_rs, k_bs, k_rs,
                  v_bs, v_rs, o_bs, o_rs, do_bs, do_rs, dq_bs, dq_rs, dk_bs, dk_rs, dv_bs, dv_rs, scale, keep, keep_ld, keep_scale,
                  part=3, dq_ctx_rows=0):
    if O.dtype == F32 and dq_ctx_rows:
        raise ValueError('the fp32 attention kernels have no context-row entry')
    _attn_bwd_call('_drop', q_ptr, k_ptr, v_ptr, O, dO, LSE, Delta, dq_ptr, dk_ptr, dv_ptr,
                   (B, H, Nq, Nk, dqk, dv, q_bs, q_rs, k_bs, k_rs, v_bs, v_rs, o_bs, o_rs, do_bs, do_rs, dq_bs, dq_rs, dk_bs, dk_rs,
                    dv_bs, dv_rs), scale, part, (_ptr(keep), keep_ld, float(keep_scale)), dq_ctx_rows)


def dropout_rows(x, keep, keep_scale, B, rows, D, out, res=None, rowscale=None):
    lib = _lib.load()
    _lib.check(lib.dav_dropout_rows(_ptr(x), int(x.dtype == F32), _ptr(res), _ptr(keep), float(keep_scale), _ptr(rowscale), B, rows, D,
                                    _ptr(out), int(out.dtype == F32), _stream()), 'dav_dropout_rows')


def cast_transpose_grouped(pairs):
    if not pairs:
        return
    arr = (_lib.DavTranspose * len(pairs))()
    for q, (x, y) in zip(arr, pairs):
        q.x, q.y_bf16, q.R, q.C = _ptr(x), _ptr(y), int(x.shape[0]), int(x.shape[1])
    _lib.check(_lib.load().dav_cast_transpose_grouped(arr, len(pairs), _stream()), 'dav_cast_transpose_grouped')



KNN_TILE = 128
KNN_NARROW_K = 8
KNN_MAX_K = 64


def knn_splits(Nq, N):
    qt, nt = -(-Nq // KNN_TILE), -(-N // KNN_TILE)
    return max(1, min(nt, -(-512 // qt)))


def knn_workspace_bytes(Nq, V, k, splits):
    return splits * V * Nq * k * 8


def mean_l2n(x, out=None):
    B, L, D = x.shape
    if x.dtype != F32 or x.stride(2) != 1:
        raise ValueError('mean_l2n needs fp32 [B, L, D] with unit column stride')
    out = torch.empty(B, D, dtype=F32, device=x.device) if out is None else out
    _lib.check(_lib.load().dav_mean_l2n_f32(_ptr(x), B, L, D, x.stride(1), x.stride(0), _ptr(out), _stream()), 'dav_mean_l2n_f32')
    return out


def knn_topk(queries, banks, k, sum_view=True, splits=None, out=None, workspace=None):
    M = len(queries)
    if M != len(banks) or not 1 <= M <= 3:
        raise ValueError('knn_topk takes 1 to 3 (query, bank) pairs')
    Nq, D = queries[0].shape
    N = banks[0].shape[0]
    for t in list(queries) + list(banks):
        if t.dtype != F32 or t.dim() != 2 or t.shape[1] != D or t.stride(1) != 1:
            raise ValueError('knn_topk needs fp32 [rows, D] operands with unit column stride')
    if any(q.shape[0] != Nq or q.stride(0) != queries[0].stride(0) for q in queries) or \
            any(x.shape[0] != N or x.stride(0) != banks[0].stride(0) for x in banks):
        raise ValueError('all query (bank) tensors need the same rows and row stride')
    V = M + int(bool(sum_view))
    S = knn_splits(Nq, N) if splits is None else int(splits)
    dev = queries[0].device
    if out is None:
        out = (torch.empty(V, Nq, k, dtype=F32, device=dev), torch.empty(V, Nq, k, dtype=torch.int32, device=dev))
    nbytes = knn_workspace_bytes(Nq, V, k, S)
    if workspace is None:
        workspace = torch.empty(nbytes, dtype=torch.uint8, device=dev)
    qp = [_ptr(q) for q in queries] + [None] * (3 - M)
    xp = [_ptr(x) for x in banks] + [None] * (3 - M)
    name = 'dav_knn_topk_f32' if k <= KNN_NARROW_K else 'dav_knn_topk_wide_f32'
    _lib.check(getattr(_lib.load(), name)(qp[0], xp[0], qp[1], xp[1], qp[2], xp[2], M, Nq, N, D, queries[0].stride(0),
                                          banks[0].stride(0), int(bool(sum_view)), int(k), S, _ptr(out[0]), _ptr(out[1]),
                                          _ptr(workspace), workspace.numel() * workspace.element_size(), _stream()), name)
    return out[0], out[1].long()


def knn_vote(top_val, top_idx, labels, num_classes, k, inv_t, self_offset=-1, out=None):
    if top_val.dim() != 3 or top_val.shape != top_idx.shape or top_val.dtype != F32 or not top_val.is_contiguous():
# ... 83 lines not shown
```

deepavfusion_amd/util/misc.py:

```python
from __future__ import annotations

import contextlib
import copy
import math
import os

import torch

from .. import engine, ops
from . import distributed as dist_utils
from .flat import FlatAdamW


def get_grad_norm_(parameters, norm_type: float = 2.0) -> torch.Tensor:
    if isinstance(parameters, torch.Tensor):
        parameters = [parameters]
    grads = [p.grad.detach() for p in parameters if p.grad is not None]
    if not grads:
        return torch.tensor(0.)
    if norm_type == math.inf:
        return max(g.abs().max() for g in grads)
    return torch.norm(torch.stack([torch.norm(g, norm_type) for g in grads]), norm_type)


# ... 111 lines not shown
    return sorted({depth} | ({round(depth * ((enc_parts - s) / enc_parts) ** 2) for s in range(1, enc_parts)} - {0, depth}), reverse=True)


def micro_step_plan(accums: int, accum_iter: int, dist_active: bool):
    if accum_iter < 1 or not 0 <= accums < accum_iter:
        raise ValueError(f'micro-step {accums} of a window of {accum_iter}')
    last = accums == accum_iter - 1
    return accums == 0, last, last


class GraphedStep:

    def __init__(self, trainer: Trainer, image_shape, audio_shape, warmup: int = 2, segments: int = 0, clip_grad=None,
                 inject_noise: bool = False):
        assert trainer.accum_iter >= 1 and isinstance(trainer.optimizer, FlatAdamW)
        self.accum_iter = int(trainer.accum_iter)
        self.clip_grad = float(clip_grad) if clip_grad else None
        from .. import autograd_bridge as bridge
        self.bridge = bridge
        self.tr = trainer
        self.model = trainer.model_without_ddp
        self.opt = trainer.optimizer
        dev = self.opt.flat.flat_p.device
        self.image = torch.zeros(image_shape, device=dev)
        self.audio = torch.zeros(audio_shape, device=dev)
        self.inject_noise = bool(inject_noise)
        if self.inject_noise:
            B = image_shape[0]
            self.noise_image = torch.zeros(B, self.model.image_gs[0] * self.model.image_gs[1], device=dev)
            self.noise_audio = torch.zeros(B, self.model.audio_gs[0] * self.model.audio_gs[1], device=dev)
        self.world = dist_utils.get_world_size()
        self.reducer = trainer.model.reducer if trainer.distributed else None
        self.dist_active = self.world > 1 or (self.reducer is not None and self.reducer.force)
        if segments <= 0:
            segments = (int(os.environ.get('DAV_DP_SEGMENTS', '0')) if self.dist_active else 0) or int(os.environ.get('DAV_SEGMENTS', '0')) or (5 if self.dist_active else 1)
        enc = self.model.encoder
        vis = enc.visual if hasattr(enc, 'visual') else (enc.video if hasattr(enc, 'video') else enc.image)
        depth = len(vis.blocks)
        segments = max(1, min(segments, depth + 1))
        self.cuts = segment_cuts(depth, segments)
        self.n_seg = len(self.cuts) + 1
        saved_hook = engine._GRAD_READY
        engine.set_grad_ready_hook(None)
        side = torch.cuda.Stream()
        side.wait_stream(torch.cuda.current_stream())
        with torch.cuda.stream(side):
            for _ in range(warmup):
                self._fwd_bwd(None)
                self.opt.flat.zero_grad()
        torch.cuda.current_stream().wait_stream(side)
        torch.cuda.synchronize()

        self.graphs = [torch.cuda.CUDAGraph() for _ in range(self.n_seg)]
        self.bucket_sched = [[] for _ in range(self.n_seg)]
        seg = [0]
        pending = [len(b[2]) for b in self.reducer.buckets] if self.reducer is not None else []

        def on_ready(p):
            if self.reducer is None:
                return
            bi = self.reducer._bucket_of.get(id(p))
            if bi is not None:
                pending[bi] -= 1
                if pending[bi] == 0:
                    self.bucket_sched[seg[0]].append(bi)
        engine.set_grad_ready_hook(on_ready)

        def layer_cb(l):
            if l in self.cuts:
                self.graphs[seg[0]].capture_end()
                seg[0] += 1
                self.graphs[seg[0]].capture_begin(pool=self.graphs[0].pool(), capture_error_mode=CAPTURE_MODE)
        cap = torch.cuda.Stream()
        cap.wait_stream(torch.cuda.current_stream())
        self.opt.flat.zero_grad()
        self.keep_grad = torch.zeros_like(self.opt.keep_grad)
        self.step_scale = torch.ones(1, dtype=torch.float32, device=dev)
        self.bad_steps = torch.zeros(1, dtype=torch.int32, device=dev)
        self._presq = torch.zeros(1, dtype=torch.float32, device=dev)
        self._presq_ws = torch.zeros(1024, dtype=torch.float32, device=dev)
        accum = self.accum_iter > 1
        self.gate = torch.ones(1, dtype=torch.int32, device=dev) if accum else None
        self._sums_dirty = False
        if accum:
            self.loss_sum_image = torch.zeros((), dtype=torch.float32, device=dev)
            self.loss_sum_audio = torch.zeros((), dtype=torch.float32, device=dev)
            self.grad_norm = torch.zeros(1, dtype=torch.float32, device=dev)
        gscale = 1.0 / self.accum_iter

        def optimizer_pass():
            gnorm = None
            if self.clip_grad is not None:
                ops.l2norm(self.opt.flat.flat_g, self._presq, self._presq_ws, 1.0)
                gnorm = self._presq
            if not accum:
                ops.step_guard(self.loss_image, self.loss_audio, gnorm, self.clip_grad, 1.0, self.step_scale, self.bad_steps)
                self.opt.launch_step(fused_norm_and_zero=True, keep_grad=self.keep_grad, gscale_dev=self.step_scale)
                self.grad_norm = self.opt.sumsq.sqrt()
                return
            ops.step_guard(self.loss_sum_image, self.loss_sum_audio, gnorm, self.clip_grad, gscale, self.step_scale, self.bad_steps)
            self.opt.launch_step(grad_scale=gscale, fused_norm_and_zero=True, keep_grad=self.keep_grad, gscale_dev=self.step_scale)
            torch.mul(self.opt.sumsq.sqrt(), gscale, out=self.grad_norm)
            self.loss_sum_image.zero_()
            self.loss_sum_audio.zero_()
        kept = set()
        with torch.cuda.stream(cap):
            self.graphs[0].capture_begin(capture_error_mode=CAPTURE_MODE)
            try:
                if os.environ.get('DAV_WGRAD_OVERWRITE', '1') != '0':
                    engine.wgrad_overwrite_begin(self.gate)
                engine.WGRAD_FLUSH_LAYERS = set(self.cuts)
                engine.invalidate_weight_cache(self.model.parameters())
                engine.refresh_weight_cache(self.model)
                self.loss_image, self.loss_audio = self._fwd_bwd(layer_cb)
                if accum:
                    self.loss_sum_image.add_(self.loss_image.reshape(()))
                    self.loss_sum_audio.add_(self.loss_audio.reshape(()))
            finally:
                kept = {id(p) for p in engine.wgrad_overwrite_end()}
                engine.WGRAD_FLUSH_LAYERS = None
            if not self.dist_active and not accum:
                optimizer_pass()
            self.graphs[seg[0]].capture_end()
            self.opt_graph = None
            if self.dist_active or accum:
                self.opt_graph = torch.cuda.CUDAGraph()
                self.opt_graph.capture_begin(pool=self.graphs[0].pool(), capture_error_mode=CAPTURE_MODE)
                optimizer_pass()
                self.opt_graph.capture_end()
        torch.cuda.current_stream().wait_stream(cap)
        torch.cuda.synchronize()
        if self.reducer is not None:
            done = {bi for s in self.bucket_sched for bi in s}
            self.bucket_sched[-1] += [bi for bi in range(len(self.reducer.buckets)) if bi not in done]
        engine.set_grad_ready_hook(saved_hook)
        self.opt.flat.zero_grad()
        self.keep_grad.copy_(torch.tensor([1 if id(p) in kept else 0 for p in self.opt.flat.params], dtype=torch.uint8))
        self.kept_params = len(kept)

    def check(self):
        n = int(self.bad_steps.item())
        if n:
            raise RuntimeError(f'Loss is {float(self.loss_image + self.loss_audio)}, stopping training '
                               f'({n} captured step(s) had a non-finite loss or gradient norm; their updates were skipped)')

    def _fwd_bwd(self, layer_cb):
        B, dev = self.image.shape[0], self.image.device
        Li, La = self.model.image_gs[0] * self.model.image_gs[1], self.model.audio_gs[0] * self.model.audio_gs[1]
        if self.inject_noise:
            noise_i, noise_a = self.noise_image, self.noise_audio
        else:
            noise_i, noise_a = torch.rand(B, Li, device=dev), torch.rand(B, La, device=dev)
        with engine.ln_fuse_for(True):
            outs, tape, aux = self.bridge.avmae_fwd(self.model, self.image, self.audio, noise_i, noise_a)
        one = torch.ones((), device=dev)
        self.bridge.avmae_bwd(self.model, tape, one, one, layer_cb=layer_cb)
        return outs[0], outs[1]

    def __call__(self, image, audio, noise_image=None, noise_audio=None):
        self.image.copy_(image, non_blocking=True)
        self.audio.copy_(audio, non_blocking=True)
        if self.inject_noise:
            self.noise_image.copy_(noise_image, non_blocking=True)
            self.noise_audio.copy_(noise_audio, non_blocking=True)
        elif noise_image is not None or noise_audio is not None:
            raise ValueError('masking noise given to a step captured with inject_noise=False (it draws its own inside the graph)')
        if self.accum_iter == 1:
            self.opt.prepare_step()
            if self.reducer is not None:
                self.reducer.begin_backward()
            for s, g in enumerate(self.graphs):
                g.replay()
                if self.reducer is not None and self.dist_active:
                    self.reducer.launch_buckets(self.bucket_sched[s])
            if self.opt_graph is not None:
                self.reducer.finish()
                self.opt_graph.replay()
            self.opt.flat.stale = self.kept_params > 0
            engine.bump_fold_generation()
            self.tr.n_steps += 1
            return self.loss_image, self.loss_audio, self.grad_norm
        tr = self.tr
        write_first, reduce, optimize = micro_step_plan(tr.accums, self.accum_iter, self.dist_active)
        if write_first and self._sums_dirty:
            self.loss_sum_image.zero_()
            self.loss_sum_audio.zero_()
        self.gate.fill_(1 if write_first else 0)
        reduce = reduce and self.dist_active
        if self.reducer is not None:
            with contextlib.nullcontext() if reduce or not self.dist_active else tr.model.no_sync():
                self.reducer.begin_backward()
        for s, g in enumerate(self.graphs):
            g.replay()
            if reduce:
                self.reducer.launch_buckets(self.bucket_sched[s])
        tr.accums += 1
        self._sums_dirty = True
        self.opt.flat.stale = self.kept_params > 0
        if optimize:
            self.opt.prepare_step()
            if reduce:
                self.reducer.finish()
            self.opt_graph.replay()
            self._sums_dirty = False
            engine.bump_fold_generation()
            tr.accums = 0
            tr.n_steps += 1
        return self.loss_image, self.loss_audio, self.grad_norm


class CheckpointManager:

    NEUTRAL_SCALER = {'scale': 1.0, 'growth_factor': 2.0, 'backoff_factor': 0.5, 'growth_interval': 2000, '_growth_tracker': 0}

    def __init__(self, modules, ckpt_dir, epochs, save_freq=None):
        self.modules, self.ckpt_dir, self.epochs, self.save_freq = modules, ckpt_dir, epochs, save_freq
        self.world_size, self.rank = dist_utils.get_world_size(), dist_utils.get_rank()
        if self.rank == 0:
            os.makedirs(ckpt_dir, exist_ok=True)

    def map_location(self, state, device):
        if isinstance(state, dict):
            return {k: self.map_location(v, device) for k, v in state.items()}
        if isinstance(state, (list, tuple)):
            return type(state)(self.map_location(v, device) for v in state)
        if isinstance(state, torch.Tensor):
            return state.detach().to(device, copy=True)
        return state

    def create_state_dict(self, save_dict=None):
        state = {}
        for k, m in self.modules.items():
            if m is None:
                state[k] = None
            elif isinstance(m, torch.Tensor):
                state[k] = m.detach().clone().cpu()
            else:
                state[k] = self.map_location(m.state_dict(), 'cpu')
        state.setdefault('scaler', dict(self.NEUTRAL_SCALER))
        if save_dict is not None:
            state.update(save_dict)
        return state

    def checkpoint(self, epoch, save_dict=None, is_best=False):
        if self.rank != 0:
            return
        state = self.create_state_dict(save_dict)
        torch.save(state, os.path.join(self.ckpt_dir, 'checkpoint_latest.pth'))
        if is_best:
            torch.save(state, os.path.join(self.ckpt_dir, 'checkpoint_best.pth'))
        if self.save_freq is not None and (epoch % self.save_freq == 0 or epoch == self.epochs):
            torch.save(state, os.path.join(self.ckpt_dir, f'checkpoint_{epoch:04d}.pth'))

    def resume(self):
        path = os.path.join(self.ckpt_dir, 'checkpoint_latest.pth')
        start_epoch, metrics = 0, {}
        if not os.path.isfile(path):
            return start_epoch, metrics
        ckpt = torch.load(path, map_location='cpu')
        for k, m in self.modules.items():
            if m is None:
                continue
            if isinstance(m, torch.Tensor):
                m.data[:] = ckpt[k].data
            else:
                m.load_state_dict(ckpt[k])
        start_epoch = ckpt['epoch']
        metrics = {k: v for k, v in ckpt.items() if k not in set(self.modules.keys()) and k not in ('epoch', 'scaler')}
        engine.invalidate_weight_cache(self.modules['state_dict'].parameters())
        for m in self.modules.values():
            if isinstance(m, FlatAdamW):
                m.sync_bf16()
        return start_epoch, metrics
```

include/dav_kernels.h:

```cpp
#ifndef DAV_KERNELS_H_
#define DAV_KERNELS_H_

#include <stddef.h>
#include <stdint.h>

#ifdef __HIPCC__
#include <hip/hip_runtime.h>
#else
typedef struct ihipStream_t* hipStream_t;
#endif

#ifdef __cplusplus
extern "C" {
#endif

#define DAV_ABI_VERSION 9
int dav_abi_version(void);
int dav_build_flags(void);
const char* dav_last_error_string(void);
int dav_tune(int knob, int value);

int dav_gemm_nt_bf16(const void* A, const void* B, int M, int N, int K, int lda, int ldb, const int* a_rowmap,
                     const float* bias, int act, const void* aux, int ldaux, const float* res, int ldres,
                     const int* res_rowmap, const int* res_rows, void* C, int ldc, int c_is_bf16, const int* c_rowmap,
                     void* C2, int ldc2, int c2_mode, int beta, float alpha, int variant, hipStream_t stream);

typedef struct DavNtLn {
  const float* stats; const float* stats2; const void* A2; const float* ln_c; float eps; int a_r0, a_r1;
  float* stats_out; void* twin_out; int ld_twin;
} DavNtLn;
int dav_gemm_nt_ln_bf16(const void* A, const void* B, int M, int N, int K, int lda, int ldb, const int* a_rowmap,
                        const float* bias, int act, const void* aux, int ldaux, const float* res, int ldres,
                        const int* res_rowmap, const int* res_rows, void* C, int ldc, int c_is_bf16, const int* c_rowmap,
                        void* C2, int ldc2, int c2_mode, int beta, float alpha, int variant, const DavNtLn* ln, hipStream_t stream);

int dav_nt_issue_log(int enable, int* out, int capacity);

int dav_nt_tune_set(const int* blob, int n_ints);

int dav_gemm_tn_bf16(const void* A, const void* B, int Mc, int N, int K, int lda, int ldb, const int* a_rowmap,
                     const int* b_rowmap, float* C, int ldc, int beta, float* bias_grad, int variant, hipStream_t stream);

typedef struct DavTnProblem {
  const void* A; const void* B;
  float* C; float* bias_grad;
  int Mc, N, K, lda, ldb, ldc;
  int a_rowmap[3], b_rowmap[3];
  int flags;
} DavTnProblem;
int dav_gemm_tn_grouped_bf16(const DavTnProblem* problems, int count, hipStream_t stream);

size_t dav_gemm_tn_gang_workspace_bytes(const DavTnProblem* problems, int count);
int dav_gemm_tn_gang_bf16(const DavTnProblem* problems, int count, void* workspace, size_t workspace_bytes, hipStream_t stream);

int dav_gemm_tn_grouped_bf16_gated(const DavTnProblem* problems, int count, const int* write_gate, hipStream_t stream);
int dav_gemm_tn_gang_bf16_gated(const DavTnProblem* problems, int count, void* workspace, size_t workspace_bytes, const int* write_gate,
                                hipStream_t stream);

int dav_attn_fwd(const void* Q, const void* K, const void* V, void* O, float* LSE, int B, int H, int Nq, int Nk, int dqk,
                 int dv, long q_bs, int q_rs, long k_bs, int k_rs, long v_bs, int v_rs, long o_bs, int o_rs, float scale,
                 hipStream_t stream);
int dav_attn_bwd(const void* Q, const void* K, const void* V, const void* O, const void* dO, const float* LSE, float* Delta,
                 void* dQ, void* dK, void* dV, int B, int H, int Nq, int Nk, int dqk, int dv, long q_bs, int q_rs, long k_bs,
                 int k_rs, long v_bs, int v_rs, long o_bs, int o_rs, long do_bs, int do_rs, long dq_bs, int dq_rs, long dk_bs,
                 int dk_rs, long dv_bs, int dv_rs, float scale, hipStream_t stream);
int dav_attn_bwd_part(const void* Q, const void* K, const void* V, const void* O, const void* dO, const float* LSE, float* Delta,
                 void* dQ, void* dK, void* dV, int B, int H, int Nq, int Nk, int dqk, int dv, long q_bs, int q_rs, long k_bs,
                 int k_rs, long v_bs, int v_rs, long o_bs, int o_rs, long do_bs, int do_rs, long dq_bs, int dq_rs, long dk_bs,
                 int dk_rs, long dv_bs, int dv_rs, float scale, int part, hipStream_t stream);

int dav_attn_bwd_ctx(const void* Q, const void* K, const void* V, const void* O, const void* dO, const float* LSE, float* Delta,
                 void* dQ, void* dK, void* dV, int B, int H, int Nq, int Nk, int dqk, int dv, long q_bs, int q_rs, long k_bs,
                 int k_rs, long v_bs, int v_rs, long o_bs, int o_rs, long do_bs, int do_rs, long dq_bs, int dq_rs, long dk_bs,
                 int dk_rs, long dv_bs, int dv_rs, float scale, int dq_ctx_rows, int part, hipStream_t stream);

int dav_attn_bias_fwd(const void* Q, const void* K, const void* V, void* O, float* LSE, int B, int H, int Nq, int Nk, int dqk,
                      int dv, long q_bs, int q_rs, long k_bs, int k_rs, long v_bs, int v_rs, long o_bs, int o_rs, float scale,
                      const float* bias, int bias_nb, int bias_ld, hipStream_t stream);
int dav_attn_bias_bwd(const void* Q, const void* K, const void* V, const void* O, const void* dO, const float* LSE, float* Delta,
                      void* dQ, void* dK, void* dV, int B, int H, int Nq, int Nk, int dqk, int dv, long q_bs, int q_rs, long k_bs,
                      int k_rs, long v_bs, int v_rs, long o_bs, int o_rs, long do_bs, int do_rs, long dq_bs, int dq_rs, long dk_bs,
                      int dk_rs, long dv_bs, int dv_rs, float scale, const float* bias, int bias_nb, int bias_ld, float* dS,
                      int part, hipStream_t stream);

int dav_attn_drop_fwd(const void* Q, const void* K, const void* V, void* O, float* LSE, int B, int H, int Nq, int Nk, int dqk,
                      int dv, long q_bs, int q_rs, long k_bs, int k_rs, long v_bs, int v_rs, long o_bs, int o_rs, float scale,
                      const void* keep, int keep_ld, float keep_scale, hipStream_t stream);
int dav_attn_drop_bwd(const void* Q, const void* K, const void* V, const void* O, const void* dO, const float* LSE, float* Delta,
                      void* dQ, void* dK, void* dV, int B, int H, int Nq, int Nk, int dqk, int dv, long q_bs, int q_rs, long k_bs,
                      int k_rs, long v_bs, int v_rs, long o_bs, int o_rs, long do_bs, int do_rs, long dq_bs, int dq_rs, long dk_bs,
                      int dk_rs, long dv_bs, int dv_rs, float scale, const void* keep, int keep_ld, float keep_scale,
                      int dq_ctx_rows, int part, hipStream_t stream);

int dav_window_unfold(const void* src, int src_is_bf16, const int* rows, int B, int nW, int A, int nF, int L, int C,
                      float fusion_scale, void* out, int out_is_bf16, hipStream_t stream);
int dav_window_fold(const float* t, const int* inv, const float* res, int B, int nW, int A, int nF, int L, int C,
                    float fusion_scale, float* out, hipStream_t stream);
int dav_relpos_bias_build(const float* table, const int* index, const float* mask, int nb, int H, int A, int N, int ld, float mul,
                          float* out, hipStream_t stream);
int dav_relpos_bias_bwd(const float* dS, const int* index, int Bw, int H, int A, int N, int ld, int T, float* dtable,
                        hipStream_t stream);

int dav_layernorm_fwd(const float* x0, long x0_bs, int r0, const float* x1, long x1_bs, int r1, int B, int D,
                      const float* gamma, const float* beta, float eps, void* y_bf16, float* y_f32, float* mean, float* rstd,
                      hipStream_t stream);
int dav_layernorm_bwd(const float* x0, long x0_bs, int r0, const float* x1, long x1_bs, int r1, int B, int D,
                      const void* dy_bf16, const float* dy_f32, const float* gamma, const float* mean, const float* rstd,
                      float* dx0, long dx0_bs, int acc0, const float* res0, long res0_bs, void* dx0_bf16, long dx0_bf_bs,
                      float* dx1, long dx1_bs, int acc1, const float* res1, long res1_bs, void* dx1_bf16, long dx1_bf_bs,
                      float* dgamma, float* dbeta, void* workspace, size_t workspace_bytes, hipStream_t stream);
size_t dav_layernorm_bwd_workspace_bytes(int rows, int D);
typedef struct DavLnReduce { const void* workspace; float* dgamma; float* dbeta; int rows; int D; } DavLnReduce;
int dav_layernorm_bwd_reduce_grouped(const DavLnReduce* items, int count, hipStream_t stream);

typedef struct DavLnFold {
  const float* w; const float* gamma; const float* beta; const float* bias;
  void* w_ln_bf16; float* ln_c; float* ln_d;
  int N, K;
} DavLnFold;
int dav_ln_fold_grouped(const DavLnFold* items, int count, hipStream_t stream);
int dav_rowstats_cast(const float* x, long x_bs, int B, int rows, int D, void* twin_bf16, float* stats, hipStream_t stream);
int dav_layernorm_bwd_twin(const void* xb0, long xb0_bs, const float* st0, int r0, const void* xb1, long xb1_bs, const float* st1, int r1,
                           int B, int D, float eps, const void* dy_bf16, const float* dy_f32, const float* gamma, const float* beta,
                           float* dx0, long dx0_bs, int acc0, const float* res0, long res0_bs, void* dx0_bf16, long dx0_bf_bs,
                           float* dx1, long dx1_bs, int acc1, const float* res1, long res1_bs, void* dx1_bf16, long dx1_bf_bs,
                           void* h_out_bf16, float* dgamma, float* dbeta, void* workspace, size_t workspace_bytes, hipStream_t stream);

int dav_mask_build(const float* noise, int N, int L, int len_keep, int64_t* ids_keep, int64_t* ids_restore, float* mask,
                   int* ids_keep32, int* ids_restore32, hipStream_t stream);
int dav_patch_gather(const float* img, int B, int C, int H, int W, const int* ids_keep32, int nk, void* A_bf16, hipStream_t stream);
int dav_patch_gather3d(const float* video, int B, int C, int T, int H, int W, int pt, const int* ids_keep32, int nk,
                       void* A_bf16, hipStream_t stream);
int dav_unshuffle_fwd(const float* emb, const float* mask_token, const float* pos, const int* ids_restore32, int B, int L, int nk,
                      int D, float* out, long out_bs, int out_row_off, hipStream_t stream);
int dav_rows_gather_cast(const float* x, long x_bs, int row_off, const int* ids32, int B, int n, int D, void* out_bf16,
                         hipStream_t stream);
int dav_rows_axpy(const float* res, const float* y, const float* scale, int B, int rows, int D, float* out, hipStream_t stream);
int dav_rows_scale_cast(const float* g, const float* scale, int B, int rows, int D, void* out_bf16, hipStream_t stream);
int dav_dropout_rows(const void* in, int in_f32, const float* res, const void* keep, float keep_scale, const float* rowscale,
                     int B, int rows, int D, void* out, int out_f32, hipStream_t stream);
int dav_unshuffle_bwd_reduce(const float* dx, long dx_bs, int row_off, const int* ids_restore32, int B, int L, int nk, int D,
                             float* dpos, float* dmask_token, hipStream_t stream);

int dav_patch_mse_fwd(const float* img, const float* pred, const float* mask, int B, int C, int H, int W, int norm_pix,
                      float* loss_patch, float* tmean, float* trstd, float* loss, float* mask_sum, hipStream_t stream);
int dav_patch_mse_bwd(const float* img, const float* pred, const float* mask, const float* tmean, const float* trstd,
                      const float* mask_sum, const float* gout, int B, int C, int H, int W, void* dpred_bf16, hipStream_t stream);

int dav_pair_expand(const float* Pv, const float* Pa, int B, int nv, int na, int Wd, void* out_bf16, hipStream_t stream);
int dav_pair_reduce(const void* d_bf16, int B, int nv, int na, int Wd, void* dPv_bf16, void* dPa_bf16, hipStream_t stream);

int dav_cast_bf16(const float* x, void* y_bf16, long n, hipStream_t stream);
int dav_add_cast(const float* a, const float* b, float* out, void* out_bf16, long n, hipStream_t stream);
int dav_cast_transpose_bf16(const float* x, void* y_bf16, int R, int C, hipStream_t stream);
typedef struct DavTranspose { const float* x; void* y_bf16; int R; int C; } DavTranspose;
int dav_cast_transpose_grouped(const DavTranspose* items, int count, hipStream_t stream);
size_t dav_l2norm_workspace_bytes(long n);
int dav_l2norm(const float* x, long n, float scale, float* out, void* workspace, size_t workspace_bytes, hipStream_t stream);
int dav_adamw_flat(float* p, float* g, float* m, float* v, void* p_bf16, long n, const long* seg_end, const float* hyper,
                   int nseg, float beta1, float beta2, float eps, const float* bias_corr, float grad_scale, float* sumsq_out,
                   int zero_grad, const unsigned char* keep_grad, const float* gscale_dev, hipStream_t stream);

int dav_step_guard(const float* loss_a, const float* loss_b, const float* gnorm, float clip, float grad_scale, float* out_scale,
                   int* bad_count, hipStream_t stream);

int dav_logmel(const float* wave, int B, int S, int n_fft, int hop, int n_mels, const float* window, const float* cos_tab,
               const float* sin_tab, const float* fbank, const int* band_lo, const int* band_hi, float eps, int apply_log,
               int drop_last, float* out, hipStream_t stream);
int dav_log10_eps(const float* x, float eps, long n, float* y, hipStream_t stream);

int dav_frame_transform_u8(const uint8_t* frames, int B, int H, int W, const int* params, int S, float mean0, float mean1,
                           float mean2, float std0, float std1, float std2, float* out, hipStream_t stream);

enum { dav_resample_max_ratio = 1024 };
int dav_wave_resample_tile(int o, int n, int width);
int dav_wave_resample(const void* wave, int wave_is_i16, int B, int L, long in_rs, const float* taps_kn, int o, int n, int width,
                      const float* gain, int clamp, float* out, int out_len, long out_rs, hipStream_t stream);

int dav_mean_l2n_f32(const float* x, int B, int L, int D, long ld_row, long ld_batch, float* out, hipStream_t stream);
int dav_knn_topk_f32(const float* q0, const float* x0, const float* q1, const float* x1, const float* q2, const float* x2, int M,
                     int Nq, int N, int D, long ldq, long ldx, int sum_view, int k, int splits, float* top_val, int* top_idx,
                     void* workspace, size_t workspace_bytes, hipStream_t stream);
int dav_knn_topk_wide_f32(const float* q0, const float* x0, const float* q1, const float* x1, const float* q2, const float* x2,
                          int M, int Nq, int N, int D, long ldq, long ldx, int sum_view, int k, int splits, float* top_val,
                          int* top_idx, void* workspace, size_t workspace_bytes, hipStream_t stream);
int dav_knn_vote_f32(const float* top_val, const int* top_idx, int V, int Nq, int kk, int k, const int* labels,
                     const uint8_t* multihot, int N, int C, const float* inv_t, int self_offset, float* scores, int* pred,
                     hipStream_t stream);

int dav_gemm_nt_f32(const float* A, const float* B, int M, int N, int K, int lda, int ldb, const int* a_rowmap,
                    const float* bias, int act, const float* aux, int ldaux, const float* res, int ldres,
                    const int* res_rowmap, const int* res_rows, float* C, int ldc, const int* c_rowmap, float* C2, int ldc2,
                    int c2_mode, int beta, float alpha, int b_kn, hipStream_t stream);
int dav_gemm_tn_f32(const float* A, const float* B, int Mc, int N, int K, int lda, int ldb, const int* a_rowmap,
                    const int* b_rowmap, float* C, int ldc, int beta, float* bias_grad, hipStream_t stream);
int dav_attn_fwd_f32(const float* Q, const float* K, const float* V, float* O, float* LSE, int B, int H, int Nq, int Nk, int dqk,
                     int dv, long q_bs, int q_rs, long k_bs, int k_rs, long v_bs, int v_rs, long o_bs, int o_rs, float scale,
                     hipStream_t stream);
int dav_attn_bwd_f32(const float* Q, const float* K, const float* V, const float* O, const float* dO, const float* LSE,
                     float* Delta, float* dQ, float* dK, float* dV, int B, int H, int Nq, int Nk, int dqk, int dv, long q_bs,
                     int q_rs, long k_bs, int k_rs, long v_bs, int v_rs, long o_bs, int o_rs, long do_bs, int do_rs, long dq_bs,
                     int dq_rs, long dk_bs, int dk_rs, long dv_bs, int dv_rs, float scale, int part, hipStream_t stream);
int dav_attn_bias_fwd_f32(const float* Q, const float* K, const float* V, float* O, float* LSE, int B, int H, int Nq, int Nk,
                          int dqk, int dv, long q_bs, int q_rs, long k_bs, int k_rs, long v_bs, int v_rs, long o_bs, int o_rs,
                          float scale, const float* bias, int bias_nb, int bias_ld, hipStream_t stream);
int dav_attn_bias_bwd_f32(const float* Q, const float* K, const float* V, const float* O, const float* dO, const float* LSE,
                          float* Delta, float* dQ, float* dK, float* dV, int B, int H, int Nq, int Nk, int dqk, int dv, long q_bs,
                          int q_rs, long k_bs, int k_rs, long v_bs, int v_rs, long o_bs, int o_rs, long do_bs, int do_rs,
                          long dq_bs, int dq_rs, long dk_bs, int dk_rs, long dv_bs, int dv_rs, float scale, const float* bias,
                          int bias_nb, int bias_ld, float* dS, int part, hipStream_t stream);
int dav_attn_drop_fwd_f32(const float* Q, const float* K, const float* V, float* O, float* LSE, int B, int H, int Nq, int Nk,
                          int dqk, int dv, long q_bs, int q_rs, long k_bs, int k_rs, long v_bs, int v_rs, long o_bs, int o_rs,
                          float scale, const void* keep, int keep_ld, float keep_scale, hipStream_t stream);
int dav_attn_drop_bwd_f32(const float* Q, const float* K, const float* V, const float* O, const float* dO, const float* LSE,
                          float* Delta, float* dQ, float* dK, float* dV, int B, int H, int Nq, int Nk, int dqk, int dv, long q_bs,
                          int q_rs, long k_bs, int k_rs, long v_bs, int v_rs, long o_bs, int o_rs, long do_bs, int do_rs,
                          long dq_bs, int dq_rs, long dk_bs, int dk_rs, long dv_bs, int dv_rs, float scale, const void* keep,
                          int keep_ld, float keep_scale, int part, hipStream_t stream);
int dav_patch_gather_f32(const float* img, int B, int C, int T, int H, int W, int pt, const int* ids_keep32, int nk, float* A,
                         hipStream_t stream);
int dav_rows_gather_f32(const float* x, long x_bs, int row_off, const int* ids32, int B, int n, int D, float* out, long out_bs,
                        hipStream_t stream);
int dav_pair_expand_f32(const float* Pv, const float* Pa, int B, int nv, int na, int Wd, float* out, hipStream_t stream);
int dav_pair_reduce_f32(const float* d, int B, int nv, int na, int Wd, float* dPv, float* dPa, hipStream_t stream);
int dav_patch_mse_bwd_f32(const float* img, const float* pred, const float* mask, const float* tmean, const float* trstd,
                          const float* mask_sum, const float* gout, int B, int C, int H, int W, float* dpred, hipStream_t stream);
int dav_add_f32(const float* a, const float* b, float* out, long n, hipStream_t stream);

int dav_batch_begin(int auto_lanes);
int dav_batch_lane(void);
int dav_batch_region(int begin);
int dav_batch_skip(int steps);
int dav_batch_suspend(int on);
int dav_batch_end(void);
int dav_batch_abort(void);
int dav_batch_stats(int* recorded_ops, int* issued_launches);

#ifdef __cplusplus
}
#endif
#endif
```

Before: 2622 AV-pairs/s.

## Compute decoder tail and MAE loss only on masked rows when predictions unused

When the training step asks only for losses, the last decoder block's MLP/residual tail, the final norm, the prediction head and the patch MSE loss run only on masked (removed) token rows, which are gathered into a compact buffer. Visible-token predictions never contribute to the masked loss, so this skips their GEMMs and loss work in both forward and backward. New kernels gather and scatter the compacted rows, zero-fill gradients for the skipped rows, and compute the loss and its gradient from the compacted predictions. A GEMM config chooser for solo problems is added to pick tiles for the new odd-sized shapes. The cost is extra gather/scatter traffic and a code path that only applies when the predictions are not returned.

```diff
diff --git a/deepavfusion_amd/_lib.py b/deepavfusion_amd/_lib.py
--- a/deepavfusion_amd/_lib.py
+++ b/deepavfusion_amd/_lib.py
@@ -64,6 +64,10 @@
     'dav_unshuffle_bwd_reduce': [_p, _l, _i, _p, _i, _i, _i, _i, _p, _p, _p],
     'dav_patch_mse_fwd': [_p, _p, _p, _i, _i, _i, _i, _i, _p, _p, _p, _p, _p, _p],
     'dav_patch_mse_bwd': [_p, _p, _p, _p, _p, _p, _p, _i, _i, _i, _i, _p, _p],
+    'dav_rows_take2': [_p, _l, _p, _l, _p, _i, _i, _i, _i, _i, _p, _p, _p],
+    'dav_rows_put2': [_p, _p, _p, _i, _i, _i, _i, _i, _p, _l, _p, _l, _p],
+    'dav_patch_mse_rows_fwd': [_p, _p, _p, _i, _i, _i, _i, _i, _i, _p, _p, _p, _p, _p, _p],
+    'dav_patch_mse_rows_bwd': [_p, _p, _p, _p, _p, _p, _p, _i, _i, _i, _i, _i, _p, _p],
     'dav_pair_expand': [_p, _p, _i, _i, _i, _i, _p, _p],
     'dav_pair_reduce': [_p, _i, _i, _i, _i, _p, _p, _p],
     'dav_cast_bf16': [_p, _p, _l, _p],
@@ -166,9 +170,11 @@
 
 
 NT_TUNING_PATH = os.environ.get('DAV_NT_TUNE_FILE') or os.path.join(os.path.dirname(os.path.abspath(__file__)), 'tuning', 'nt_gfx950.json')
+NT_TUNED_LONE = {}
 
 
 def load_nt_tuning(path):
+    NT_TUNED_LONE.clear()
     if os.environ.get('DAV_NT_TUNE', '1') == '0' or not path or not os.path.exists(path):
         _lib.dav_nt_tune_set(None, 0)
         return 0
@@ -178,6 +184,8 @@
         blob += [int(e['cfg']), int(e['b_kn']), len(e['problems'])]
         for q in e['problems']:
             blob += [int(x) for x in q]
+        if len(e['problems']) == 1:
+            NT_TUNED_LONE[(int(e['b_kn']), *(int(x) for x in e['problems'][0]))] = int(e['cfg'])
     arr = (C.c_int * len(blob))(*blob)
     n = _lib.dav_nt_tune_set(arr, len(blob))
     if n < 0:
diff --git a/deepavfusion_amd/autograd_bridge.py b/deepavfusion_amd/autograd_bridge.py
--- a/deepavfusion_amd/autograd_bridge.py
+++ b/deepavfusion_amd/autograd_bridge.py
@@ -446,12 +446,29 @@
     return _FusionBlockFn.apply(fb, c(xmm), c(xv), c(xa), *list(fb.parameters()))
 
 
-def avmae_fwd(model, image, audio, noise_i, noise_a):
+def avmae_fwd(model, image, audio, noise_i, noise_a, losses_only=False):
     with E.fold_scope(model):
-        return _avmae_fwd(model, image, audio, noise_i, noise_a)
-
-
-def _avmae_fwd(model, image, audio, noise_i, noise_a):
+        return _avmae_fwd(model, image, audio, noise_i, noise_a, losses_only)
+
+
+def _dec_loss_fwd(target, pred, t_d, mask, norm_loss):
+    if t_d.get('removed', False):
+        return E.loss_fwd_removed(target, pred, t_d['ids_restore32'], t_d['nk'], norm_loss)
+    return E.loss_fwd(target, pred, mask, norm_loss)
+
+
+def _dec_loss_bwd(target, pred, mask, t_l, t_d, g_l, g_p):
+    if t_d.get('removed', False):
+        if g_p is not None:
+            raise ValueError('a gradient for the predictions of a losses_only forward (it returned none)')
+        return E.loss_bwd_removed(target, pred, t_l, g_l)
+    dp = E.loss_bwd(target, pred, mask, t_l, g_l)
+    if g_p is not None:
+        dp = (dp.float() + g_p.reshape(dp.shape)).to(E.BF16)
+    return dp
+
+
+def _avmae_fwd(model, image, audio, noise_i, noise_a, losses_only=False):
     enc = model.encoder
     B = image.shape[0]
     Li, La = model.image_gs[0] * model.image_gs[1], model.audio_gs[0] * model.audio_gs[1]
@@ -462,15 +479,16 @@
     nF = enc.fusion_tokens.shape[1]
     dec_i, dec_a = model.decoder('image'), model.decoder('audio')
     main, sa, _ = _streams(image.device)
+    mro = losses_only and E.decoder_trim_ok(dec_i, nki, Li) and E.decoder_trim_ok(dec_a, nka, La)
     lanes = t_enc['lanes']
     if lanes:
         with E.batch() as bt:
             bt.lane()
-            pred_i, t_di = E.decoder_fwd(dec_i, xi_b, xf_b, ir32, B, nki, nF)
-            loss_i, t_li = E.loss_fwd(image, pred_i, im, model.image_norm_loss)
+            pred_i, t_di = E.decoder_fwd(dec_i, xi_b, xf_b, ir32, B, nki, nF, masked_rows_only=mro)
+            loss_i, t_li = _dec_loss_fwd(image, pred_i, t_di, im, model.image_norm_loss)
             bt.lane()
-            pred_a, t_da = E.decoder_fwd(dec_a, xa_b, xf_b, ar32, B, nka, nF)
-            loss_a, t_la = E.loss_fwd(audio, pred_a, am, model.audio_norm_loss)
+            pred_a, t_da = E.decoder_fwd(dec_a, xa_b, xf_b, ar32, B, nka, nF, masked_rows_only=mro)
+            loss_a, t_la = _dec_loss_fwd(audio, pred_a, t_da, am, model.audio_norm_loss)
     else:
         si = main
         sa.wait_stream(main)
@@ -478,8 +496,8 @@
             si.wait_stream(main)
 
         def chain(dec, x_b, r32, nk, target, mask, norm_loss):
-            pred, t_d = yield from E.decoder_fwd_steps(dec, x_b, xf_b, r32, B, nk, nF)
-            loss, t_l = E.loss_fwd(target, pred, mask, norm_loss)
+            pred, t_d = yield from E.decoder_fwd_steps(dec, x_b, xf_b, r32, B, nk, nF, masked_rows_only=mro)
+            loss, t_l = _dec_loss_fwd(target, pred, t_d, mask, norm_loss)
             return pred, t_d, loss, t_l
         (pred_a, t_da, loss_a, t_la), (pred_i, t_di, loss_i, t_li) = paired_steps(
             chain(dec_a, xa_b, ar32, nka, audio, am, model.audio_norm_loss), sa,
@@ -490,6 +508,8 @@
     tape = dict(image=image, audio=audio, im=im, am=am, ik32=ik32, ak32=ak32, dec_lanes=lanes, t_enc=t_enc, t_di=t_di, t_da=t_da, t_li=t_li,
                 t_la=t_la, pred_i=pred_i, pred_a=pred_a, B=B)
     aux = dict(image_ids_keep=ik, image_mask=im, image_ids_restore=ir, audio_ids_keep=ak, audio_mask=am, audio_ids_restore=ar)
+    if losses_only:
+        return (loss_i, loss_a, None, None), tape, aux
     return (loss_i, loss_a, pred_i, pred_a), tape, aux
 
 
@@ -501,19 +521,16 @@
     B = t['B']
     dec_i, dec_a = model.decoder('image'), model.decoder('audio')
     main, sa, _ = _streams(t['image'].device)
+    mro = lambda t_d: t_d.get('removed', False)
     if t['dec_lanes']:
-        dpi = E.loss_bwd(t['image'], t['pred_i'], t['im'], t['t_li'], g_li)
-        dpa = E.loss_bwd(t['audio'], t['pred_a'], t['am'], t['t_la'], g_la)
-        if g_pi is not None:
-            dpi = (dpi.float() + g_pi.reshape(dpi.shape)).to(E.BF16)
-        if g_pa is not None:
-            dpa = (dpa.float() + g_pa.reshape(dpa.shape)).to(E.BF16)
+        dpi = _dec_loss_bwd(t['image'], t['pred_i'], t['im'], t['t_li'], t['t_di'], g_li, g_pi)
+        dpa = _dec_loss_bwd(t['audio'], t['pred_a'], t['am'], t['t_la'], t['t_da'], g_la, g_pa)
         with E.deferred_wgrads():
             with E.batch() as bt:
                 bt.lane()
-                dxi_b, dxf_i = E.decoder_bwd(dec_i, t['t_di'], dpi, t['ik32'], B)
-                bt.lane()
-                dxa_b, dxf_a = E.decoder_bwd(dec_a, t['t_da'], dpa, t['ak32'], B)
+                dxi_b, dxf_i = E.decoder_bwd(dec_i, t['t_di'], dpi, t['ik32'], B, masked_rows_only=mro(t['t_di']))
+                bt.lane()
+                dxa_b, dxf_a = E.decoder_bwd(dec_a, t['t_da'], dpa, t['ak32'], B, masked_rows_only=mro(t['t_da']))
     elif _DEC_WGRAD_JOINT and sa is not main:
         with E.deferred_wgrads():
             si = main
@@ -522,10 +539,8 @@
                 si.wait_stream(main)
 
             def chain(dec, target, pred, mask, t_l, g_l, g_p, t_d, k32):
-                dp = E.loss_bwd(target, pred, mask, t_l, g_l)
-                if g_p is not None:
-                    dp = (dp.float() + g_p.reshape(dp.shape)).to(E.BF16)
-                return (yield from E.decoder_bwd_steps(dec, t_d, dp, k32, B))
+                dp = _dec_loss_bwd(target, pred, mask, t_l, t_d, g_l, g_p)
+                return (yield from E.decoder_bwd_steps(dec, t_d, dp, k32, B, masked_rows_only=mro(t_d)))
             (dxa_b, dxf_a), (dxi_b, dxf_i) = paired_steps(
                 chain(dec_a, t['audio'], t['pred_a'], t['am'], t['t_la'], g_la, g_pa, t['t_da'], t['ak32']), sa,
                 chain(dec_i, t['image'], t['pred_i'], t['im'], t['t_li'], g_li, g_pi, t['t_di'], t['ik32']), si, DEC_JOIN)
@@ -536,15 +551,11 @@
     else:
         sa.wait_stream(main)
         with torch.cuda.stream(sa), E.deferred_wgrads():
-            dpa = E.loss_bwd(t['audio'], t['pred_a'], t['am'], t['t_la'], g_la)
-            if g_pa is not None:
-                dpa = (dpa.float() + g_pa.reshape(dpa.shape)).to(E.BF16)
-            dxa_b, dxf_a = E.decoder_bwd(dec_a, t['t_da'], dpa, t['ak32'], B)
+            dpa = _dec_loss_bwd(t['audio'], t['pred_a'], t['am'], t['t_la'], t['t_da'], g_la, g_pa)
+            dxa_b, dxf_a = E.decoder_bwd(dec_a, t['t_da'], dpa, t['ak32'], B, masked_rows_only=mro(t['t_da']))
         with E.deferred_wgrads():
-            dpi = E.loss_bwd(t['image'], t['pred_i'], t['im'], t['t_li'], g_li)
-            if g_pi is not None:
-                dpi = (dpi.float() + g_pi.reshape(dpi.shape)).to(E.BF16)
-            dxi_b, dxf_i = E.decoder_bwd(dec_i, t['t_di'], dpi, t['ik32'], B)
+            dpi = _dec_loss_bwd(t['image'], t['pred_i'], t['im'], t['t_li'], t['t_di'], g_li, g_pi)
+            dxi_b, dxf_i = E.decoder_bwd(dec_i, t['t_di'], dpi, t['ik32'], B, masked_rows_only=mro(t['t_di']))
         main.wait_stream(sa)
     dxf32 = dxf_i.float() + dxf_a.float()
     if layer_cb is not None:
diff --git a/deepavfusion_amd/csrc/dectail/dectail.hip b/deepavfusion_amd/csrc/dectail/dectail.hip
--- /dev/null
+++ b/deepavfusion_amd/csrc/dectail/dectail.hip
@@ -0,0 +1,211 @@
+#include "common.h"
+#include "dav_kernels.h"
+
+namespace {
+
+__device__ __forceinline__ int compact_row(int r, int nk, int L) { return (r >= nk && r < L) ? r - nk : -1; }
+
+__global__ __launch_bounds__(256) void rows_take2_kernel(const bf16_t* __restrict__ o, long o_bs, const float* __restrict__ x, long x_bs,
+                                                         const int* __restrict__ restore, int B, int nF, int L, int nk, int D,
+                                                         bf16_t* __restrict__ o_c, float* __restrict__ x_c) {
+  const int lane = threadIdx.x & 63;
+  const int gw = (blockIdx.x * blockDim.x + threadIdx.x) >> 6, nwaves = (gridDim.x * blockDim.x) >> 6;
+  const int nm = L - nk, n8 = D >> 3, n4 = D >> 2;
+  for (int row = gw; row < B * L; row += nwaves) {
+    const int b = row / L, j = row % L;
+    const int c = compact_row(restore[row], nk, L);
+    if (c < 0) continue;
+    const long src = (long)(nF + j) * D, dst = ((long)b * nm + c) * D;
+    const uint4* so = reinterpret_cast<const uint4*>(o + b * o_bs + src);
+    uint4* to = reinterpret_cast<uint4*>(o_c + dst);
+    for (int i = lane; i < n8; i += 64) to[i] = so[i];
+    const float4* sx = reinterpret_cast<const float4*>(x + b * x_bs + src);
+    float4* tx = reinterpret_cast<float4*>(x_c + dst);
+    for (int i = lane; i < n4; i += 64) tx[i] = sx[i];
+  }
+}
+
+__global__ __launch_bounds__(256) void rows_put2_kernel(const bf16_t* __restrict__ do_c, const float* __restrict__ g1_c,
+                                                        const int* __restrict__ restore, int B, int nF, int L, int nk, int D,
+                                                        bf16_t* __restrict__ dout, long do_bs, float* __restrict__ g1, long g1_bs) {
+  const int lane = threadIdx.x & 63;
+  const int gw = (blockIdx.x * blockDim.x + threadIdx.x) >> 6, nwaves = (gridDim.x * blockDim.x) >> 6;
+  const int R = nF + L, nm = L - nk, n8 = D >> 3, n4 = D >> 2;
+  for (int row = gw; row < B * R; row += nwaves) {
+    const int b = row / R, r = row % R;
+    const int c = r < nF ? -1 : compact_row(restore[b * L + r - nF], nk, L);
+    uint4* to = reinterpret_cast<uint4*>(dout + b * do_bs + (long)r * D);
+    float4* tx = reinterpret_cast<float4*>(g1 + b * g1_bs + (long)r * D);
+    if (c < 0) {
+      for (int i = lane; i < n8; i += 64) to[i] = uint4{0u, 0u, 0u, 0u};
+      for (int i = lane; i < n4; i += 64) tx[i] = float4{0.f, 0.f, 0.f, 0.f};
+      continue;
+    }
+    const long src = ((long)b * nm + c) * D;
+    const uint4* so = reinterpret_cast<const uint4*>(do_c + src);
+    for (int i = lane; i < n8; i += 64) to[i] = so[i];
+    const float4* sx = reinterpret_cast<const float4*>(g1_c + src);
+    for (int i = lane; i < n4; i += 64) tx[i] = sx[i];
+  }
+}
+
+template <int C>
+__global__ __launch_bounds__(256) void patch_mse_rows_fwd_kernel(const float* __restrict__ img, const float* __restrict__ pred_c,
+                                                                 const int* __restrict__ restore, int B, int H, int W, int nk,
+                                                                 int norm_pix, float* __restrict__ loss_patch_c,
+                                                                 float* __restrict__ tmean_c, float* __restrict__ trstd_c) {
+  constexpr int P = 256 * C, PER = P / 64;
+  const int lane = threadIdx.x & 63;
+  const int gw = (blockIdx.x * blockDim.x + threadIdx.x) >> 6, nwaves = (gridDim.x * blockDim.x) >> 6;
+  const int gW = W >> 4, L = (H >> 4) * gW, nm = L - nk;
+  for (int row = gw; row < B * L; row += nwaves) {
+    const int b = row / L, l = row % L, gy = l / gW, gx = l % gW;
+    const int c_ = compact_row(restore[row], nk, L);
+    if (c_ < 0) continue;
+    const long crow = (long)b * nm + c_;
+    float t[PER];
+    float s = 0.f;
+#pragma unroll
+    for (int k = 0; k < PER; ++k) {
+      const int e = lane + 64 * k, pix = e / C, c = e % C;
+      t[k] = img[(((long)b * C + c) * H + gy * 16 + (pix >> 4)) * W + gx * 16 + (pix & 15)];
+      s += t[k];
+    }
+    float mean = 0.f, rstd = 1.f;
+    if (norm_pix) {
+      mean = wave_sum(s) / P;
+      float q = 0.f;
+#pragma unroll
+      for (int k = 0; k < PER; ++k) q += (t[k] - mean) * (t[k] - mean);
+      rstd = 1.f / sqrtf(wave_sum(q) / (P - 1) + 1.e-6f);
+    }
+    float acc = 0.f;
+#pragma unroll
+    for (int k = 0; k < PER; ++k) {
+      const float d = pred_c[crow * P + lane + 64 * k] - (t[k] - mean) * rstd;
+      acc += d * d;
+    }
+    acc = wave_sum(acc) / P;
+    if (lane == 0) { loss_patch_c[crow] = acc; tmean_c[crow] = mean; trstd_c[crow] = rstd; }
+  }
+}
+
+__global__ __launch_bounds__(1024) void removed_mean_kernel(const float* __restrict__ loss_patch_c, const int* __restrict__ restore, int B,
+                                                            int L, int nk, float* __restrict__ out, float* __restrict__ mask_sum) {
+  __shared__ float sa[16], sb[16];
+  const int nm = L - nk;
+  float a = 0.f, m = 0.f;
+  for (int i = threadIdx.x; i < B * L; i += blockDim.x) {
+    const int c = compact_row(restore[i], nk, L);
+    if (c >= 0) { a += loss_patch_c[(long)(i / L) * nm + c]; m += 1.f; }
+  }
+  a = wave_sum(a); m = wave_sum(m);
+  if ((threadIdx.x & 63) == 0) { sa[threadIdx.x >> 6] = a; sb[threadIdx.x >> 6] = m; }
+  __syncthreads();
+  if (threadIdx.x == 0) {
+    float ta = 0.f, tb = 0.f;
+    for (int i = 0; i < (int)(blockDim.x >> 6); ++i) { ta += sa[i]; tb += sb[i]; }
+    out[0] = ta / tb;
+    mask_sum[0] = tb;
+  }
+}
+
+template <int C>
+__global__ __launch_bounds__(256) void patch_mse_rows_bwd_kernel(const float* __restrict__ img, const float* __restrict__ pred_c,
+                                                                 const int* __restrict__ restore, const float* __restrict__ tmean_c,
+                                                                 const float* __restrict__ trstd_c, const float* __restrict__ mask_sum,
+                                                                 const float* __restrict__ gout, int B, int H, int W, int nk,
+                                                                 bf16_t* __restrict__ dpred_c) {
+  constexpr int P = 256 * C, PER = P / 64;
+  const int lane = threadIdx.x & 63;
+  const int gw = (blockIdx.x * blockDim.x + threadIdx.x) >> 6, nwaves = (gridDim.x * blockDim.x) >> 6;
+  const int gW = W >> 4, L = (H >> 4) * gW, nm = L - nk;
+  const float coef = (gout ? gout[0] : 1.f) * 2.f / (P * mask_sum[0]);
+  for (int row = gw; row < B * L; row += nwaves) {
+    const int b = row / L, l = row % L, gy = l / gW, gx = l % gW;
+    const int c_ = compact_row(restore[row], nk, L);
+    if (c_ < 0) continue;
+    const long crow = (long)b * nm + c_;
+    const float m = 1.f * coef, mean = tmean_c[crow], rstd = trstd_c[crow];
+#pragma unroll
+    for (int k = 0; k < PER; ++k) {
+      const int e = lane + 64 * k, pix = e / C, c = e % C;
+      const float t = img[(((long)b * C + c) * H + gy * 16 + (pix >> 4)) * W + gx * 16 + (pix & 15)];
+      dpred_c[crow * P + e] = f2bf(m * (pred_c[crow * P + e] - (t - mean) * rstd));
+    }
+  }
+}
+
+int wave_grid(long rows) {
+  long g = (rows + 3) / 4;
+  return (int)(g > 2048 ? 2048 : (g < 1 ? 1 : g));
+}
+
+bool rows_shape_ok(int B, int nF, int L, int nk, int D, long bs0, long bs1) {
+  if (B <= 0 || nF < 0 || L <= 0 || nk <= 0 || nk >= L || D <= 0 || (D & 7)) return false;
+  const long need = (long)(nF + L) * D;
+  return bs0 >= need && bs1 >= need && (long)B * (nF + L) < (1l << 31);
+}
+
+bool mse_shape_ok(int B, int C, int H, int W, int nk) {
+  if (B <= 0 || H <= 0 || W <= 0 || (H & 15) || (W & 15) || (C != 1 && C != 3)) return false;
+  const long L = (long)(H >> 4) * (W >> 4);
+  return nk > 0 && nk < L && B * L < (1l << 31);
+}
+
+}
+
+extern "C" int dav_rows_take2(const void* o_bf16, long o_bs, const float* x, long x_bs, const int* ids_restore32, int B, int nF, int L,
+                              int nk, int D, void* o_c_bf16, float* x_c, hipStream_t stream) {
+  if (!rows_shape_ok(B, nF, L, nk, D, o_bs, x_bs)) return DAV_ERR_SHAPE;
+  if (!o_bf16 || !x || !ids_restore32 || !o_c_bf16 || !x_c) return DAV_ERR_SHAPE;
+  if ((((uintptr_t)o_bf16 | (uintptr_t)x | (uintptr_t)o_c_bf16 | (uintptr_t)x_c) & 15) || ((uintptr_t)ids_restore32 & 3) ||
+      (o_bs & 7) || (x_bs & 3))
+    return DAV_ERR_ALIGN;
+  DAV_LAUNCH(rows_take2_kernel, dim3(wave_grid((long)B * L)), dim3(256), 0, stream, (const bf16_t*)o_bf16, o_bs, x, x_bs, ids_restore32,
+             B, nF, L, nk, D, (bf16_t*)o_c_bf16, x_c);
+  return dav_launch_status();
+}
+
+extern "C" int dav_rows_put2(const void* do_c_bf16, const float* g1_c, const int* ids_restore32, int B, int nF, int L, int nk, int D,
+                             void* do_bf16, long do_bs, float* g1, long g1_bs, hipStream_t stream) {
+  if (!rows_shape_ok(B, nF, L, nk, D, do_bs, g1_bs)) return DAV_ERR_SHAPE;
+  if (!do_c_bf16 || !g1_c || !ids_restore32 || !do_bf16 || !g1) return DAV_ERR_SHAPE;
+  if ((((uintptr_t)do_c_bf16 | (uintptr_t)g1_c | (uintptr_t)do_bf16 | (uintptr_t)g1) & 15) || ((uintptr_t)ids_restore32 & 3) ||
+      (do_bs & 7) || (g1_bs & 3))
+    return DAV_ERR_ALIGN;
+  DAV_LAUNCH(rows_put2_kernel, dim3(wave_grid((long)B * (nF + L))), dim3(256), 0, stream, (const bf16_t*)do_c_bf16, g1_c, ids_restore32,
+             B, nF, L, nk, D, (bf16_t*)do_bf16, do_bs, g1, g1_bs);
+  return dav_launch_status();
+}
+
+extern "C" int dav_patch_mse_rows_fwd(const float* img, const float* pred_c, const int* ids_restore32, int B, int C, int H, int W,
+                                      int nk, int norm_pix, float* loss_patch_c, float* tmean_c, float* trstd_c, float* loss,
+                                      float* mask_sum, hipStream_t stream) {
+  if (!mse_shape_ok(B, C, H, W, nk)) return DAV_ERR_SHAPE;
+  if (!img || !pred_c || !ids_restore32 || !loss_patch_c || !tmean_c || !trstd_c || !loss || !mask_sum) return DAV_ERR_SHAPE;
+  if (((uintptr_t)pred_c & 15) || (((uintptr_t)img | (uintptr_t)ids_restore32 | (uintptr_t)loss_patch_c | (uintptr_t)tmean_c |
+                                    (uintptr_t)trstd_c | (uintptr_t)loss | (uintptr_t)mask_sum) & 3))
+    return DAV_ERR_ALIGN;
+  const int L = (H >> 4) * (W >> 4);
+  const dim3 grid(wave_grid((long)B * L));
+  if (C == 3) DAV_LAUNCH(patch_mse_rows_fwd_kernel<3>, grid, dim3(256), 0, stream, img, pred_c, ids_restore32, B, H, W, nk, norm_pix, loss_patch_c, tmean_c, trstd_c);
+  else DAV_LAUNCH(patch_mse_rows_fwd_kernel<1>, grid, dim3(256), 0, stream, img, pred_c, ids_restore32, B, H, W, nk, norm_pix, loss_patch_c, tmean_c, trstd_c);
+  DAV_LAUNCH(removed_mean_kernel, dim3(1), dim3(1024), 0, stream, loss_patch_c, ids_restore32, B, L, nk, loss, mask_sum);
+  return dav_launch_status();
+}
+
+extern "C" int dav_patch_mse_rows_bwd(const float* img, const float* pred_c, const int* ids_restore32, const float* tmean_c,
+                                      const float* trstd_c, const float* mask_sum, const float* gout, int B, int C, int H, int W,
+                                      int nk, void* dpred_c_bf16, hipStream_t stream) {
+  if (!mse_shape_ok(B, C, H, W, nk)) return DAV_ERR_SHAPE;
+  if (!img || !pred_c || !ids_restore32 || !tmean_c || !trstd_c || !mask_sum || !dpred_c_bf16) return DAV_ERR_SHAPE;
+  if ((((uintptr_t)pred_c | (uintptr_t)dpred_c_bf16) & 15) || (((uintptr_t)img | (uintptr_t)ids_restore32 | (uintptr_t)tmean_c |
+                                                                (uintptr_t)trstd_c | (uintptr_t)mask_sum | (uintptr_t)gout) & 3))
+    return DAV_ERR_ALIGN;
+  const int L = (H >> 4) * (W >> 4);
+  const dim3 grid(wave_grid((long)B * L));
+  if (C == 3) DAV_LAUNCH(patch_mse_rows_bwd_kernel<3>, grid, dim3(256), 0, stream, img, pred_c, ids_restore32, tmean_c, trstd_c, mask_sum, gout, B, H, W, nk, (bf16_t*)dpred_c_bf16);
+  else DAV_LAUNCH(patch_mse_rows_bwd_kernel<1>, grid, dim3(256), 0, stream, img, pred_c, ids_restore32, tmean_c, trstd_c, mask_sum, gout, B, H, W, nk, (bf16_t*)dpred_c_bf16);
+  return dav_launch_status();
+}
diff --git a/deepavfusion_amd/engine.py b/deepavfusion_amd/engine.py
--- a/deepavfusion_amd/engine.py
+++ b/deepavfusion_amd/engine.py
@@ -519,8 +519,15 @@
         _DEFERRED_LN_READY.append((norm.weight, norm.bias))
 
 
+def _nt_variant_like(like_M, N, K, flags, b_kn):
+    if like_M is None or PRECISION == 'fp32':
+        return 0
+    cfg = ops.nt_lone_config(like_M, N, K, flags, b_kn)
+    return cfg << 4 if cfg in ops.NT_EXPLICIT_CFGS else 0
+
+
 def lin_fwd(lin, a, M, *, a_rowmap=None, lda=None, act=0, res=None, res_rowmap=None, out=None, out_bf16=False,
-            c_rowmap=None, ldc=None, C2=None, c2_mode=0, w_col_off=0, k=None, use_bias=True):
+            c_rowmap=None, ldc=None, C2=None, c2_mode=0, w_col_off=0, k=None, use_bias=True, like_M=None):
     W = wcache(lin.weight)
     N, Kfull = W.shape
     K = Kfull if k is None else k
@@ -528,16 +535,17 @@
     if out is None:
         out = _e((M, N), BF16 if out_bf16 else F32, dev)
     Bw = W if w_col_off == 0 else W.view(-1)[w_col_off:]
+    flags = act | (4 if out.dtype == BF16 else 0) | (8 if res is not None else 0) | ((c2_mode << 4) if C2 is not None else 0)
     ops.gemm_nt(a, Bw, M, N, K, lda=lda if lda is not None else K, ldb=Kfull, a_rowmap=a_rowmap,
                 bias=lin.bias if use_bias else None, act=act, res=res, ldres=N, res_rowmap=res_rowmap,
                 C_out=out, ldc=ldc if ldc is not None else N, c_bf16=out.dtype == BF16, c_rowmap=c_rowmap,
-                C2=C2, ldc2=N, c2_mode=c2_mode)
+                C2=C2, ldc2=N, c2_mode=c2_mode, variant=_nt_variant_like(like_M, N, K, flags, 0))
     return out
 
 
 def lin_bwd(lin, dy, a, M, *, dy_rowmap=None, a_rowmap=None, lda=None, need_dx=True, gelu_aux=None, dx=None, dx_bf16=True,
             dx_rowmap=None, dx_beta=0, dx_C2=None, dx_c2_mode=0, w_col_off=0, k=None, use_bias=True, final=True,
-            dx_res=None, dx_res_rowmap=None, wgrad=True):
+            dx_res=None, dx_res_rowmap=None, wgrad=True, like_M=None):
     W = wcache(lin.weight)
     N, Kfull = W.shape
     K = Kfull if k is None else k
@@ -550,6 +558,10 @@
         else:
             WT = wcache_t(lin.weight)
             Bt, ldb, variant = (WT if w_col_off == 0 else WT[w_col_off:]), N, 0
+        if like_M is not None:
+            flags = ((3 if gelu_aux is not None else 0) | (4 if dx.dtype == BF16 else 0) | (8 if dx_res is not None else 0)
+                     | ((dx_c2_mode << 4) if dx_C2 is not None else 0) | (256 if dx_beta else 0))
+            variant |= _nt_variant_like(like_M, K, N, flags, variant >> 12)
         ops.gemm_nt(dy, Bt, M, K, N, lda=N, ldb=ldb, a_rowmap=dy_rowmap, act=3 if gelu_aux is not None else 0,
                     aux=gelu_aux, ldaux=K, res=dx_res, ldres=K, res_rowmap=dx_res_rowmap,
                     C_out=dx, ldc=K, c_bf16=dx.dtype == BF16, c_rowmap=dx_rowmap, beta=dx_beta,
@@ -1391,27 +1403,97 @@
         return e.value
 
 
-def decoder_fwd(dec, x_b, xf_b, ids_restore32, B, nk, nF):
-    return drain(decoder_fwd_steps(dec, x_b, xf_b, ids_restore32, B, nk, nF))
-
-
-def decoder_fwd_steps(dec, x_b, xf_b, ids_restore32, B, nk, nF):
+DEC_TRIM = os.environ.get('DAV_DEC_TRIM', '0') == '1'
+
+
+def set_dec_trim(on: bool):
+    global DEC_TRIM
+    DEC_TRIM = bool(on)
+
+
+def _block_drops_something(blk) -> bool:
+    return any((isinstance(m, torch.nn.Dropout) and m.p > 0) or getattr(m, 'drop_prob', 0.0) for m in blk.modules()) and blk.training
+
+
+def decoder_trim_ok(dec, nk, L) -> bool:
+    Dd = dec.embed.weight.shape[0]
+    return (DEC_TRIM and getattr(dec, 'arch', 'plain') != 'swin' and PRECISION == 'bf16' and not ln_fuse_ok(Dd) and Dd % 8 == 0
+            and 0 < nk < L and len(dec.blocks) > 0 and not _block_drops_something(dec.blocks[-1]))
+
+
+def _block_fwd_removed(blk, x, heads, eps, ids_restore32, nk, nF):
+    B, R, D = x.shape
+    L, hd, dev = R - nF, D // heads, x.device
+    nm = L - nk
+    M, Mc = B * R, B * nm
+    h1, _, st1 = ln_fwd(blk.norm1, None, x, B, eps)
+    qkv = lin_fwd(blk.attn.qkv, h1, M, out_bf16=True)
+    o, lse = attention_fwd(*qkv_cols(qkv, R, D), B, heads, R, R, hd, hd, hd ** -0.5)
+    o_c, x_c = _e((Mc, D), BF16, dev), _e((B, nm, D), F32, dev)
+    ops.rows_take2(o, R * D, x, R * D, ids_restore32, B, nF, L, nk, D, o_c, x_c)
+    x1 = lin_fwd(blk.attn.proj, o_c, Mc, res=x_c, like_M=M).view(B, nm, D)
+    h2, _, st2 = ln_fwd(blk.norm2, None, x1, B, eps)
+    Hd = blk.mlp.fc1.weight.shape[0]
+    z = _e((Mc, Hd), BF16, dev)
+    u = lin_fwd(blk.mlp.fc1, h2, Mc, act=1, out_bf16=True, C2=z, c2_mode=4, like_M=M)
+    x2 = lin_fwd(blk.mlp.fc2, u, Mc, res=x1, like_M=M).view(B, nm, D)
+    tape = dict(x_mod=x, x_fus=None, h1=h1, st1=st1, qkv=qkv, o=o, lse=lse, o_c=o_c, x1=x1, h2=h2, st2=st2, z=z, u=u, heads=heads, nF=0)
+    return x2, tape
+
+
+def _block_bwd_removed(blk, t, g2, g2b, ids_restore32, nk, nF):
+    x = t['x_mod']
+    B, R, D = x.shape
+    L, heads, dev = R - nF, t['heads'], x.device
+    hd, nm = D // heads, L - nk
+    M, Mc = B * R, B * nm
+    dz = lin_bwd(blk.mlp.fc2, g2b, t['u'], Mc, gelu_aux=t['z'], like_M=M)
+    g1_c, g1b_c = _e((B, nm, D), F32, dev), _e((Mc, D), BF16, dev)
+    dh2 = lin_bwd(blk.mlp.fc1, dz, t['h2'], Mc, like_M=M)
+    ln_bwd(blk.norm2, None, t['x1'], B, t['st2'], dy_bf16=dh2, dx1=g1_c, res1=g2, dx1_bf16=g1b_c)
+    do_c = lin_bwd(blk.attn.proj, g1b_c, t['o_c'], Mc, like_M=M)
+    do, g1 = _e((M, D), BF16, dev), _e((B, R, D), F32, dev)
+    ops.rows_put2(do_c, g1_c, ids_restore32, B, nF, L, nk, D, do, R * D, g1, R * D)
+    dqkv = _e((M, 3 * D), BF16, dev)
+    attention_bwd(*qkv_cols(t['qkv'], R, D), t['o'], do, t['lse'], *qkv_cols(dqkv, R, D), B, heads, R, R, hd, hd, hd ** -0.5)
+    dh1 = lin_bwd(blk.attn.qkv, dqkv, t['h1'], M)
+    dx, dxb, _ = block_bwd_tail(blk, t, dict(dh1=dh1, g1=g1))
+    return dx, dxb
+
+
+def decoder_fwd(dec, x_b, xf_b, ids_restore32, B, nk, nF, masked_rows_only=False):
+    return drain(decoder_fwd_steps(dec, x_b, xf_b, ids_restore32, B, nk, nF, masked_rows_only=masked_rows_only))
+
+
+def decoder_fwd_steps(dec, x_b, xf_b, ids_restore32, B, nk, nF, masked_rows_only=False):
     L = ids_restore32.shape[1]
     Dd = dec.embed.weight.shape[0]
     dev = x_b.device
+    removed = masked_rows_only and decoder_trim_ok(dec, nk, L)
     emb = lin_fwd(dec.embed, x_b, B * nk)
     x = _e((B, nF + L, Dd), F32, dev)
     lin_fwd(dec.embed, xf_b, B * nF, out=x, c_rowmap=(nF, nF + L, 0))
     ops.unshuffle_fwd(emb, dec.mask_token, dec.pos_embed, ids_restore32, B, L, nk, Dd, x, (nF + L) * Dd, nF)
     tapes = []
     swin = getattr(dec, 'arch', 'plain') == 'swin'
-    for blk in dec.blocks:
+    for i, blk in enumerate(dec.blocks):
         if swin:
             x, bt = swin_block_fwd(blk, x, nF)
+        elif removed and i == len(dec.blocks) - 1:
+            x, bt = _block_fwd_removed(blk, x, dec.heads, blk.norm1.eps, ids_restore32, nk, nF)
         else:
             x, bt = block_fwd(blk, x, None, dec.heads, blk.norm1.eps)
         tapes.append(bt)
         yield
+    if removed:
+        nm = L - nk
+        hN = _e((B * nm, Dd), BF16, dev)
+        mean, rstd = _e((B * nm,), F32, dev), _e((B * nm,), F32, dev)
+        ops.layernorm_fwd(x, nm * Dd, nm, None, 0, 0, B, Dd, dec.norm.weight, dec.norm.bias, dec.norm.eps, hN, None, mean, rstd)
+        pred = lin_fwd(dec.pred, hN, B * nm, like_M=B * L)
+        tape = dict(x_b=x_b, xf_b=xf_b, x_last=x, tapes=tapes, hN=hN, stN=(mean, rstd), ids_restore32=ids_restore32, nk=nk, nF=nF, L=L,
+                    removed=True)
+        return pred.view(B, nm, pred.shape[1]), tape
     D_ = Dd
     if not swin and ln_fuse_ok(Dd):
         tw_last = ensure_tw(x)
@@ -1429,39 +1511,51 @@
     return pred.view(B, L, P), tape
 
 
-def decoder_bwd(dec, t, dpred_b, ids_keep32, B):
-    return drain(decoder_bwd_steps(dec, t, dpred_b, ids_keep32, B))
-
-
-def decoder_bwd_steps(dec, t, dpred_b, ids_keep32, B):
+def decoder_bwd(dec, t, dpred_b, ids_keep32, B, masked_rows_only=False):
+    return drain(decoder_bwd_steps(dec, t, dpred_b, ids_keep32, B, masked_rows_only=masked_rows_only))
+
+
+def decoder_bwd_steps(dec, t, dpred_b, ids_keep32, B, masked_rows_only=False):
     nk, nF, L = t['nk'], t['nF'], t['L']
     Dd = dec.embed.weight.shape[0]
     dev = dpred_b.device
+    removed = t.get('removed', False)
+    if removed and not masked_rows_only:
+        raise ValueError('decoder tape of the removed-patch tail given to a backward that was not asked for it')
     fused = t.get('ln_fused', False)
-    dhN = lin_bwd(dec.pred, dpred_b, None if fused else t['hN'], B * L, wgrad=not fused)
-    g = _e((B, nF + L, Dd), F32, dev)
-    gb = _e((B * (nF + L), Dd), BF16, dev)
-    g[:, :nF].zero_()
-    gb.view(B, nF + L, Dd)[:, :nF].zero_()
-    if fused:
-        xb, st = t['tw_last']
-        hN = _e((B * L, Dd), BF16, dev)
-        ops.layernorm_bwd_twin((xb, nF * Dd), (nF + L) * Dd, (st, nF * (Dd // 64) * 2), L, None, 0, None, 0, B, Dd, dec.norm.eps,
-                               dhN, None, dec.norm.weight, dec.norm.bias,
-                               (g, nF * Dd), (nF + L) * Dd, 0, None, 0, (gb, nF * Dd), (nF + L) * Dd,
-                               h_out=hN, dgamma=gbuf(dec.norm.weight), dbeta=gbuf(dec.norm.bias))
-        lin_wgrad(dec.pred, dpred_b, hN, B * L)
+    if removed:
+        nm = L - nk
+        dhN = lin_bwd(dec.pred, dpred_b, t['hN'], B * nm, like_M=B * L)
+        g, gb = _e((B, nm, Dd), F32, dev), _e((B * nm, Dd), BF16, dev)
+        ops.layernorm_bwd(t['x_last'], nm * Dd, nm, None, 0, 0, B, Dd, dhN, None, dec.norm.weight, t['stN'][0], t['stN'][1],
+                          g, nm * Dd, 0, None, 0, gb, nm * Dd, None, 0, 0, None, 0, None, 0, gbuf(dec.norm.weight), gbuf(dec.norm.bias))
     else:
-        xs = t['x_last'].view(-1)[nF * Dd:]
-        ops.layernorm_bwd(xs, (nF + L) * Dd, L, None, 0, 0, B, Dd, dhN, None, dec.norm.weight, t['stN'][0], t['stN'][1],
-                          g.view(-1)[nF * Dd:], (nF + L) * Dd, 0, None, 0, gb.view(-1)[nF * Dd:], (nF + L) * Dd,
-                          None, 0, 0, None, 0, None, 0, gbuf(dec.norm.weight), gbuf(dec.norm.bias))
+        dhN = lin_bwd(dec.pred, dpred_b, None if fused else t['hN'], B * L, wgrad=not fused)
+        g = _e((B, nF + L, Dd), F32, dev)
+        gb = _e((B * (nF + L), Dd), BF16, dev)
+        g[:, :nF].zero_()
+        gb.view(B, nF + L, Dd)[:, :nF].zero_()
+        if fused:
+            xb, st = t['tw_last']
+            hN = _e((B * L, Dd), BF16, dev)
+            ops.layernorm_bwd_twin((xb, nF * Dd), (nF + L) * Dd, (st, nF * (Dd // 64) * 2), L, None, 0, None, 0, B, Dd, dec.norm.eps,
+                                   dhN, None, dec.norm.weight, dec.norm.bias,
+                                   (g, nF * Dd), (nF + L) * Dd, 0, None, 0, (gb, nF * Dd), (nF + L) * Dd,
+                                   h_out=hN, dgamma=gbuf(dec.norm.weight), dbeta=gbuf(dec.norm.bias))
+            lin_wgrad(dec.pred, dpred_b, hN, B * L)
+        else:
+            xs = t['x_last'].view(-1)[nF * Dd:]
+            ops.layernorm_bwd(xs, (nF + L) * Dd, L, None, 0, 0, B, Dd, dhN, None, dec.norm.weight, t['stN'][0], t['stN'][1],
+                              g.view(-1)[nF * Dd:], (nF + L) * Dd, 0, None, 0, gb.view(-1)[nF * Dd:], (nF + L) * Dd,
+                              None, 0, 0, None, 0, None, 0, gbuf(dec.norm.weight), gbuf(dec.norm.bias))
     _ready(dec.norm.weight, dec.norm.bias)
     swin = getattr(dec, 'arch', 'plain') == 'swin'
     yield
-    for blk, bt in zip(reversed(list(dec.blocks)), reversed(t['tapes'])):
+    for i, (blk, bt) in enumerate(zip(reversed(list(dec.blocks)), reversed(t['tapes']))):
         if swin:
             g, gb = swin_block_bwd(blk, bt, g, gb)
+        elif removed and i == 0:
+            g, gb = _block_bwd_removed(blk, bt, g, gb, t['ids_restore32'], nk, nF)
         else:
             g, gb, _ = block_bwd(blk, bt, g, gb)
         yield
@@ -1553,3 +1647,19 @@
     dpred = _e((B * L, P), BF16, img.device)
     ops.patch_mse_bwd(img, pred, mask, t['tm'], t['tr'], t['msum'], gout, dpred)
     return dpred
+
+
+def loss_fwd_removed(img, pred_c, ids_restore32, nk, norm_pix):
+    B, nm, _ = pred_c.shape
+    dev = img.device
+    lp, tm, tr = _e((B * nm,), F32, dev), _e((B * nm,), F32, dev), _e((B * nm,), F32, dev)
+    loss, msum = _e((1,), F32, dev), _e((1,), F32, dev)
+    ops.patch_mse_rows_fwd(img, pred_c, ids_restore32, nk, norm_pix, lp, tm, tr, loss, msum)
+    return loss.view(()), dict(tm=tm, tr=tr, msum=msum, lp=lp, ids_restore32=ids_restore32, nk=nk)
+
+
+def loss_bwd_removed(img, pred_c, t, gout):
+    B, nm, P = pred_c.shape
+    dpred = _e((B * nm, P), BF16, img.device)
+    ops.patch_mse_rows_bwd(img, pred_c, t['ids_restore32'], t['nk'], t['tm'], t['tr'], t['msum'], gout, dpred)
+    return dpred
diff --git a/deepavfusion_amd/ops.py b/deepavfusion_amd/ops.py
--- a/deepavfusion_amd/ops.py
+++ b/deepavfusion_amd/ops.py
@@ -180,6 +180,25 @@
         out.append((cfg, bt, probs, flags) if with_flags else (cfg, bt, probs))
         i += 3 + 4 * cnt
     return out
+
+
+NT_EXPLICIT_CFGS = (3, 5, 7, 8, 43, 44, 45, 46)
+
+
+def nt_lone_config(M, N, K, flags, b_kn):
+    _lib.load()
+    cfg = _lib.NT_TUNED_LONE.get((int(bool(b_kn)), M, N, K, flags))
+    if cfg is not None:
+        return cfg
+    rows = (M + 127) // 128
+    t128 = rows * ((N + 127) // 128)
+    if N <= 64 or t128 < 100:
+        return 5
+    if t128 < 400:
+        return 8
+    if K <= 512 and N % 256 == 0 and N >= 1024 and rows * ((N + 255) // 256) >= 512:
+        return 44
+    return 3
 
 
 def gemm_tn(A, B, Mc, N, K, C_out, *, lda=None, ldb=None, ldc=None, a_rowmap=None, b_rowmap=None, beta=1, bias_grad=None,
@@ -455,6 +474,32 @@
         return
     _lib.check(lib.dav_patch_mse_bwd(_ptr(img), _ptr(pred), _ptr(mask), _ptr(tmean), _ptr(trstd), _ptr(mask_sum), _ptr(gout),
                                      B, Cc, H, W, _ptr(dpred_bf16), _stream()), 'dav_patch_mse_bwd')
+
+
+def rows_take2(o, o_bs, x, x_bs, ids_restore32, B, nF, L, nk, D, o_c, x_c):
+    lib = _lib.load()
+    _lib.check(lib.dav_rows_take2(_ptr(o), o_bs, _ptr(x), x_bs, _ptr(ids_restore32), B, nF, L, nk, D, _ptr(o_c), _ptr(x_c), _stream()),
+               'dav_rows_take2')
+
+
+def rows_put2(do_c, g1_c, ids_restore32, B, nF, L, nk, D, do, do_bs, g1, g1_bs):
+    lib = _lib.load()
+    _lib.check(lib.dav_rows_put2(_ptr(do_c), _ptr(g1_c), _ptr(ids_restore32), B, nF, L, nk, D, _ptr(do), do_bs, _ptr(g1), g1_bs, _stream()),
+               'dav_rows_put2')
+
+
+def patch_mse_rows_fwd(img, pred_c, ids_restore32, nk, norm_pix, loss_patch_c, tmean_c, trstd_c, loss, mask_sum):
+    lib = _lib.load()
+    B, Cc, H, W = img.shape
+    _lib.check(lib.dav_patch_mse_rows_fwd(_ptr(img), _ptr(pred_c), _ptr(ids_restore32), B, Cc, H, W, nk, int(norm_pix), _ptr(loss_patch_c),
+                                          _ptr(tmean_c), _ptr(trstd_c), _ptr(loss), _ptr(mask_sum), _stream()), 'dav_patch_mse_rows_fwd')
+
+
+def patch_mse_rows_bwd(img, pred_c, ids_restore32, nk, tmean_c, trstd_c, mask_sum, gout, dpred_c_bf16):
+    lib = _lib.load()
+    B, Cc, H, W = img.shape
+    _lib.check(lib.dav_patch_mse_rows_bwd(_ptr(img), _ptr(pred_c), _ptr(ids_restore32), _ptr(tmean_c), _ptr(trstd_c), _ptr(mask_sum),
+                                          _ptr(gout), B, Cc, H, W, nk, _ptr(dpred_c_bf16), _stream()), 'dav_patch_mse_rows_bwd')
 
 
 def pair_expand(Pv, Pa, B, nv, na, Wd, out):
diff --git a/deepavfusion_amd/util/misc.py b/deepavfusion_amd/util/misc.py
--- a/deepavfusion_amd/util/misc.py
+++ b/deepavfusion_amd/util/misc.py
@@ -287,7 +287,7 @@
         else:
             noise_i, noise_a = torch.rand(B, Li, device=dev), torch.rand(B, La, device=dev)
         with engine.ln_fuse_for(True):
-            outs, tape, aux = self.bridge.avmae_fwd(self.model, self.image, self.audio, noise_i, noise_a)
+            outs, tape, aux = self.bridge.avmae_fwd(self.model, self.image, self.audio, noise_i, noise_a, losses_only=True)
         one = torch.ones((), device=dev)
         self.bridge.avmae_bwd(self.model, tape, one, one, layer_cb=layer_cb)
         return outs[0], outs[1]
diff --git a/include/dav_kernels.h b/include/dav_kernels.h
--- a/include/dav_kernels.h
+++ b/include/dav_kernels.h
@@ -146,6 +146,17 @@
                       float* loss_patch, float* tmean, float* trstd, float* loss, float* mask_sum, hipStream_t stream);
 int dav_patch_mse_bwd(const float* img, const float* pred, const float* mask, const float* tmean, const float* trstd,
                       const float* mask_sum, const float* gout, int B, int C, int H, int W, void* dpred_bf16, hipStream_t stream);
+
+int dav_rows_take2(const void* o_bf16, long o_bs, const float* x, long x_bs, const int* ids_restore32, int B, int nF, int L, int nk,
+                   int D, void* o_c_bf16, float* x_c, hipStream_t stream);
+int dav_rows_put2(const void* do_c_bf16, const float* g1_c, const int* ids_restore32, int B, int nF, int L, int nk, int D,
+                  void* do_bf16, long do_bs, float* g1, long g1_bs, hipStream_t stream);
+int dav_patch_mse_rows_fwd(const float* img, const float* pred_c, const int* ids_restore32, int B, int C, int H, int W, int nk,
+                           int norm_pix, float* loss_patch_c, float* tmean_c, float* trstd_c, float* loss, float* mask_sum,
+                           hipStream_t stream);
+int dav_patch_mse_rows_bwd(const float* img, const float* pred_c, const int* ids_restore32, const float* tmean_c, const float* trstd_c,
+                           const float* mask_sum, const float* gout, int B, int C, int H, int W, int nk, void* dpred_c_bf16,
+                           hipStream_t stream);
 
 int dav_pair_expand(const float* Pv, const float* Pa, int B, int nv, int na, int Wd, void* out_bf16, hipStream_t stream);
 int dav_pair_reduce(const void* d_bf16, int B, int nv, int na, int Wd, void* dPv_bf16, void* dPa_bf16, hipStream_t stream);
```

Result: no change. 2624 AV-pairs/s (median of 2 runs) (+0.1%).
